# Duankaiwen/LSNet

Hardware: AMD Instinct MI355X
Metric: img/s train LSNet R-50-FPN 1333x800 bs2/GPU (higher is better)
Workload: dtype f32 (fp32-equivalent: 6 bf16 MFMA terms per product on exact 3-way operand splits, fp32 accumulate); 1 GPU; LSNet R50-FPN bbox (conv_module_type=dcn), 2 img/GPU 3x800x1344 (1333x800 padded to /32), 7 gt/img, fwd+bwd+gradient arena (the reducer's buckets, no collective on one rank)+clip35+SGD; global_batch=2, parallelism=dp1, world_size=1, memory_format=channels_last, launch=eager

## Files before the change

### include/lsnet_hip.h

```cpp
#ifndef LSNET_HIP_H_
#define LSNET_HIP_H_

#include <stdint.h>

#ifdef __cplusplus
extern "C" {
#endif

typedef struct ihipStream_t *lsn_stream_t;

typedef enum {
    LSN_OK = 0,
    LSN_ERR_INVALID = -1,
    LSN_ERR_UNSUPPORTED = -2,
    LSN_ERR_RUNTIME = -3
} lsn_status;

typedef enum { LSN_NCHW = 0, LSN_NHWC = 1 } lsn_layout;

typedef struct { int64_t b, c, h, w; } lsn_strides4;

typedef struct {
    int B, C, H, W;
    int Co, Ho, Wo;
    int kh, kw, stride, pad, dil;
    int groups, deformable_groups;
    float scale_h, scale_w;
    int mask_is_logit;
    void *workspace;
    void *gather_workspace;
    int64_t gather_workspace_bytes;
    int accumulate_param_grads;
    int out_pitch;
    int weights_prepared;
} lsn_dcn_shape;

typedef struct {
    const float *input;
    const float *offset;
    const float *mask;
    float *output;
    const float *grad_output;
    float *grad_input;
    float *grad_offset;
    float *grad_mask;
    lsn_strides4 off_st, mask_st;
    int B, H, W, Ho, Wo;
    float scale_h, scale_w;
} lsn_dcn_level;

const char *lsn_last_error(void);
int lsn_version(void);

enum { LSN_MATH_FP32 = 0, LSN_MATH_BF16X3 = 1, LSN_MATH_BF16X6 = 2, LSN_MATH_BF16 = 3 };
int lsn_set_math_mode(int mode);
int lsn_get_math_mode(void);


#define LSN_DCN_KD_EVERY_ROUTE 55

int lsn_dcn_forward(const lsn_dcn_shape *shape, int n_levels, const lsn_dcn_level *levels,
                    const float *weight, const float *bias, lsn_layout layout, lsn_stream_t stream);

int lsn_dcn_backward(const lsn_dcn_shape *shape, int n_levels, const lsn_dcn_level *levels,
                     const float *weight, float *grad_weight, float *grad_bias, lsn_layout layout,
                     lsn_stream_t stream);

int64_t lsn_dcn_backward_workspace_bytes(const lsn_dcn_shape *shape, int n_levels, const lsn_dcn_level *levels);
int lsn_dcn_pitched_ok(const lsn_dcn_shape *shape, int n_levels, const lsn_dcn_level *levels, int backward);
int lsn_dcn_prepared_ok(const lsn_dcn_shape *shape, int n_levels, const lsn_dcn_level *levels, int backward);
int lsn_dcn_anchor_lists(const lsn_dcn_shape *shape, int n_levels, const lsn_dcn_level *levels, lsn_layout layout,
                         int *sample_anchor, int *list_start, int *list_sample, int64_t *counts, lsn_stream_t stream);


int lsn_deform_conv_forward(const float *input, const float *weight, const float *offset, float *output,
                            int B, int C, int H, int W, int Co, int kW, int kH, int dW, int dH, int padW,
                            int padH, int dilW, int dilH, int group, int deformable_group,
                            int im2col_step, lsn_stream_t stream);
int lsn_deform_conv_backward_input(const float *input, const float *offset, const float *grad_output,
                                   float *grad_input, float *grad_offset, const float *weight, int B,
                                   int C, int H, int W, int Co, int kW, int kH, int dW, int dH, int padW,
                                   int padH, int dilW, int dilH, int group, int deformable_group,
                                   int im2col_step, lsn_stream_t stream);
int lsn_deform_conv_backward_parameters(const float *input, const float *offset, const float *grad_output,
                                        float *grad_weight, int B, int C, int H, int W, int Co, int kW,
                                        int kH, int dW, int dH, int padW, int padH, int dilW, int dilH,
                                        int group, int deformable_group, float scale, int im2col_step,
                                        lsn_stream_t stream);
int lsn_modulated_deform_conv_forward(const float *input, const float *weight, const float *bias,
                                      const float *offset, const float *mask, float *output, int B, int C,
                                      int H, int W, int Co, int kernel_h, int kernel_w, int stride_h,
                                      int stride_w, int pad_h, int pad_w, int dilation_h, int dilation_w,
                                      int group, int deformable_group, int with_bias, lsn_stream_t stream);
int lsn_modulated_deform_conv_backward(const float *input, const float *weight, const float *bias,
                                       const float *offset, const float *mask, float *grad_input,
                                       float *grad_weight, float *grad_bias, float *grad_offset,
                                       float *grad_mask, const float *grad_output, int B, int C, int H,
                                       int W, int Co, int kernel_h, int kernel_w, int stride_h,
                                       int stride_w, int pad_h, int pad_w, int dilation_h, int dilation_w,
                                       int group, int deformable_group, int with_bias,
                                       lsn_stream_t stream);
int lsn_pyramid_deform_conv_forward(const float *input, const float *weight, const float *offset,
                                    float *output, int B, int C, int H, int W, int Co, int Ho, int Wo,
                                    int kW, int kH, int dW, int dH, int padW, int padH, int dilW, int dilH,
                                    float scaleW, float scaleH, int group, int deformable_group,
                                    int im2col_step, lsn_stream_t stream);
int lsn_pyramid_deform_conv_backward_input(const float *input, const float *offset,
                                           const float *grad_output, float *grad_input,
                                           float *grad_offset, const float *weight, int B, int C, int H,
                                           int W, int Co, int Ho, int Wo, int kW, int kH, int dW, int dH,
                                           int padW, int padH, int dilW, int dilH, float scaleW,
                                           float scaleH, int group, int deformable_group,
                                           int im2col_step, lsn_stream_t stream);
int lsn_pyramid_deform_conv_backward_parameters(const float *input, const float *offset,
                                                const float *grad_output, float *grad_weight, int B,
                                                int C, int H, int W, int Co, int Ho, int Wo, int kW,
                                                int kH, int dW, int dH, int padW, int padH, int dilW,
                                                int dilH, float scaleW, float scaleH, int group,
                                                int deformable_group, float scale, int im2col_step,
                                                lsn_stream_t stream);

int lsn_sigmoid_focal_loss_forward(const float *logits, const int64_t *targets, float *losses, int N,
                                   int C, float gamma, float alpha, lsn_stream_t stream);
// ... 344 lines not shown
```

### lsnet_amd/_lib.py

```python
import ctypes
import os

_HERE = os.path.dirname(os.path.abspath(__file__))
SO_PATH = os.environ.get('LSNET_HIP_SO') or os.path.join(_HERE, 'csrc', 'liblsnet_hip.so')


class Strides4(ctypes.Structure):
    c_name = 'lsn_strides4'
    _fields_ = [('b', ctypes.c_int64), ('c', ctypes.c_int64), ('h', ctypes.c_int64), ('w', ctypes.c_int64)]


class DcnShape(ctypes.Structure):
    c_name = 'lsn_dcn_shape'
    _fields_ = [('B', ctypes.c_int), ('C', ctypes.c_int), ('H', ctypes.c_int), ('W', ctypes.c_int),
                ('Co', ctypes.c_int), ('Ho', ctypes.c_int), ('Wo', ctypes.c_int),
                ('kh', ctypes.c_int), ('kw', ctypes.c_int), ('stride', ctypes.c_int), ('pad', ctypes.c_int),
                ('dil', ctypes.c_int), ('groups', ctypes.c_int), ('deformable_groups', ctypes.c_int),
                ('scale_h', ctypes.c_float), ('scale_w', ctypes.c_float), ('mask_is_logit', ctypes.c_int),
                ('workspace', ctypes.c_void_p), ('gather_workspace', ctypes.c_void_p),
                ('gather_workspace_bytes', ctypes.c_int64), ('accumulate_param_grads', ctypes.c_int),
                ('out_pitch', ctypes.c_int), ('weights_prepared', ctypes.c_int)]


class DcnLevel(ctypes.Structure):
    c_name = 'lsn_dcn_level'
    _fields_ = [('input', ctypes.c_void_p), ('offset', ctypes.c_void_p), ('mask', ctypes.c_void_p),
                ('output', ctypes.c_void_p), ('grad_output', ctypes.c_void_p), ('grad_input', ctypes.c_void_p),
                ('grad_offset', ctypes.c_void_p), ('grad_mask', ctypes.c_void_p),
                ('off_st', Strides4), ('mask_st', Strides4),
                ('B', ctypes.c_int), ('H', ctypes.c_int), ('W', ctypes.c_int), ('Ho', ctypes.c_int),
                ('Wo', ctypes.c_int), ('scale_h', ctypes.c_float), ('scale_w', ctypes.c_float)]


class OffsetChainLevel(ctypes.Structure):
    c_name = 'lsn_offset_chain_level'
    _fields_ = [('off', ctypes.c_void_p), ('out', ctypes.c_void_p * 3), ('gout', ctypes.c_void_p * 6), ('goff', ctypes.c_void_p),
                ('images', ctypes.c_int64), ('per_image', ctypes.c_int64), ('off_image_pitch', ctypes.c_int64),
                ('mh', ctypes.c_float * 3), ('mw', ctypes.c_float * 3)]


class WgradBnJob(ctypes.Structure):
    c_name = 'lsn_wgrad_bn_job'
    _fields_ = [('x', ctypes.c_void_p), ('g', ctypes.c_void_p), ('w', ctypes.c_void_p), ('bn_gamma', ctypes.c_void_p),
                ('bn_mean', ctypes.c_void_p), ('bn_var', ctypes.c_void_p), ('bn_eps', ctypes.c_float),
                ('grad_w', ctypes.c_void_p), ('grad_gamma', ctypes.c_void_p), ('grad_beta', ctypes.c_void_p)]


class SgdTensor(ctypes.Structure):
    c_name = 'lsn_sgd_tensor'
    _fields_ = [('param', ctypes.c_void_p), ('grad', ctypes.c_void_p), ('momentum_buf', ctypes.c_void_p),
                ('numel', ctypes.c_int64), ('first_chunk', ctypes.c_int64), ('group', ctypes.c_int)]


class SgdGroup(ctypes.Structure):
    c_name = 'lsn_sgd_group'
    _fields_ = [('lr', ctypes.c_float), ('momentum', ctypes.c_float), ('weight_decay', ctypes.c_float)]


class ConvLevel(ctypes.Structure):
    c_name = 'lsn_conv_level'
    _fields_ = [('x', ctypes.c_void_p), ('out', ctypes.c_void_p), ('grad_out', ctypes.c_void_p),
                ('B', ctypes.c_int), ('H', ctypes.c_int), ('W', ctypes.c_int), ('residual', ctypes.c_void_p),
                ('gate', ctypes.c_void_p)]


class ConvWprep(ctypes.Structure):
    c_name = 'lsn_conv_wprep'
    _fields_ = [('kind', ctypes.c_int), ('w', ctypes.c_void_p), ('prepared', ctypes.c_void_p), ('C', ctypes.c_int),
                ('Co', ctypes.c_int), ('kh', ctypes.c_int), ('kw', ctypes.c_int), ('stride', ctypes.c_int),
                ('pad', ctypes.c_int), ('dil', ctypes.c_int),
                ('bn_gamma', ctypes.c_void_p), ('bn_var', ctypes.c_void_p), ('bn_beta', ctypes.c_void_p),
                ('bn_mean', ctypes.c_void_p), ('shift_out', ctypes.c_void_p), ('bn_eps', ctypes.c_float)]


class GnLevel(ctypes.Structure):
    c_name = 'lsn_gn_level'
    _fields_ = [('x', ctypes.c_void_p), ('y', ctypes.c_void_p), ('dy', ctypes.c_void_p), ('dx', ctypes.c_void_p),
                ('B', ctypes.c_int), ('HW', ctypes.c_int), ('y_batch_stride', ctypes.c_longlong),
                ('dy_batch_stride', ctypes.c_longlong)]


class GateJob(ctypes.Structure):
    c_name = 'lsn_gate_job'
    _fields_ = [('grad_y', ctypes.c_void_p), ('y', ctypes.c_void_p), ('grad', ctypes.c_void_p), ('B', ctypes.c_int),
# ... 8 lines not shown


class DecodeSource(ctypes.Structure):
    c_name = 'lsn_decode_source'
    _fields_ = [('H', ctypes.c_int), ('W', ctypes.c_int), ('stride', ctypes.c_float),
                ('heat', ctypes.c_void_p), ('offset', ctypes.c_void_p),
                ('heat_strides', ctypes.c_int64 * 4), ('offset_strides', ctypes.c_int64 * 4)]


class CornerLevel(ctypes.Structure):
    c_name = 'lsn_corner_level'
    _fields_ = [('H', ctypes.c_int), ('W', ctypes.c_int), ('score', ctypes.c_void_p), ('offset', ctypes.c_void_p),
                ('score_strides', ctypes.c_int64 * 4), ('offset_strides', ctypes.c_int64 * 4),
                ('grad_score', ctypes.c_void_p), ('grad_offset', ctypes.c_void_p),
                ('grad_score_strides', ctypes.c_int64 * 4), ('grad_offset_strides', ctypes.c_int64 * 4)]


class SemLevel(ctypes.Structure):
    c_name = 'lsn_sem_level'
    _fields_ = [('H', ctypes.c_int), ('W', ctypes.c_int), ('logits', ctypes.c_void_p), ('strides', ctypes.c_int64 * 4),
                ('grad', ctypes.c_void_p), ('grad_strides', ctypes.c_int64 * 4)]


class ProfEntry(ctypes.Structure):
    c_name = 'lsn_prof_entry'
    _fields_ = [('name', ctypes.c_char * 48), ('launches', ctypes.c_longlong), ('total_ms', ctypes.c_double),
                ('flops', ctypes.c_double), ('bytes', ctypes.c_double)]


class ProfLaunch(ctypes.Structure):
    c_name = 'lsn_prof_launch'
    _fields_ = [(k, ctypes.c_int) for k in ('kind', 'C', 'Co', 'kh', 'kw', 'stride', 'pad', 'dil', 'relu', 'xpitch', 'n_levels',
                                            'has_residual', 'has_gate')] + \
               [('B', ctypes.c_int * 16), ('H', ctypes.c_int * 16), ('W', ctypes.c_int * 16), ('ms', ctypes.c_float)]


STRUCTS = (Strides4, DcnShape, DcnLevel, OffsetChainLevel, WgradBnJob, SgdTensor, SgdGroup, ConvLevel, ConvWprep, GnLevel, GateJob,
           DecodeLevel, DecodeSource, CornerLevel, SemLevel, ProfEntry, ProfLaunch)


def _signatures():
    i, q, f, d, p, c_char_p, P = ctypes.c_int, ctypes.c_int64, ctypes.c_float, ctypes.c_double, ctypes.c_void_p, \
        ctypes.c_char_p, ctypes.POINTER
    return {
        'lsn_last_error': (c_char_p, []),
        'lsn_version': (i, []),
        'lsn_set_math_mode': (i, [i]),
        'lsn_get_math_mode': (i, []),
        'lsn_dcn_forward': (i, [P(DcnShape), i, P(DcnLevel), p, p, i, p]),
        'lsn_dcn_backward': (i, [P(DcnShape), i, P(DcnLevel), p, p, p, i, p]),
        'lsn_dcn_backward_workspace_bytes': (q, [P(DcnShape), i, P(DcnLevel)]),
        'lsn_dcn_pitched_ok': (i, [P(DcnShape), i, P(DcnLevel), i]),
        'lsn_dcn_prepared_ok': (i, [P(DcnShape), i, P(DcnLevel), i]),
        'lsn_dcn_anchor_lists': (i, [P(DcnShape), i, P(DcnLevel), i, p, p, p, p, p]),
        'lsn_deform_conv_forward': (i, [p] * 4 + [i] * 16 + [p]),
        'lsn_deform_conv_backward_input': (i, [p] * 6 + [i] * 16 + [p]),
        'lsn_deform_conv_backward_parameters': (i, [p] * 4 + [i] * 15 + [f, i, p]),
        'lsn_modulated_deform_conv_forward': (i, [p] * 6 + [i] * 16 + [p]),
        'lsn_modulated_deform_conv_backward': (i, [p] * 11 + [i] * 16 + [p]),
        'lsn_pyramid_deform_conv_forward': (i, [p] * 4 + [i] * 15 + [f, f, i, i, i, p]),
        'lsn_pyramid_deform_conv_backward_input': (i, [p] * 6 + [i] * 15 + [f, f, i, i, i, p]),
        'lsn_pyramid_deform_conv_backward_parameters': (i, [p] * 4 + [i] * 15 + [f, f, i, i, f, i, p]),
        'lsn_sigmoid_focal_loss_forward': (i, [p, p, p, i, i, f, f, p]),
        'lsn_sigmoid_focal_loss_backward': (i, [p] * 4 + [i, i, f, f, p]),
        'lsn_sigmoid_focal_loss_sum': (i, [p] * 4 + [i, i, f, f, p]),
        'lsn_sigmoid_focal_loss_backward_weighted': (i, [p] * 5 + [i, i, f, f, p]),
        'lsn_sigmoid_focal_loss_level_sums': (i, [p] * 4 + [i] * 4 + [p, f, f, p]),
        'lsn_sigmoid_focal_loss_backward_levels': (i, [p] * 5 + [i] * 4 + [p, f, f, p]),
        'lsn_level_sums': (i, [p, p, i, i, i, p, p]),
        'lsn_level_expand': (i, [p, p, i, i, i, p, p]),
        'lsn_clip_sgd_workspace_bytes': (q, []),
        'lsn_clip_sgd_step': (i, [i, p, q, i, P(SgdGroup), f, p, p, p]),
        'lsn_offset_chain_forward': (i, [i, P(OffsetChainLevel), i, p]),
        'lsn_offset_chain_backward': (i, [i, P(OffsetChainLevel), i, p]),
        'lsn_topk_columns': (i, [p] + [i] * 4 + [p, p, i, i, p, p, p]),
        'lsn_assign_workspace_bytes': (q, [i] * 4),
        'lsn_centroid_assign': (i, [p, i, p, p, i, f, i] + [p] * 5),
        'lsn_centroid_assign_batch': (i, [p, i, p, p, i, p, f, i] + [p] * 5),
        'lsn_atss_assign': (i, [p, i, i, i, p, p, i, i] + [p] * 6),
        'lsn_atss_assign_batch': (i, [p, i, i, i, p, p, i, p, i] + [p] * 6),
        'lsn_dense_targets': (i, [p, i, p, i, p, p]),
        'lsn_centroid_assign_masked_batch': (i, [p, i, p, p, p, i, p, f, i] + [p] * 5),
        'lsn_atss_assign_masked_batch': (i, [p, i, i, i, p, p, p, i, p, i] + [p] * 6),
        'lsn_assign_targets_batch': (i, [p, p, i, i, p, p, i, p, q] + [p] * 6),
        'lsn_nms_workspace_bytes': (q, [i]),
        'lsn_nms': (i, [p, p, i, f] + [p] * 4),
        'lsn_conv2d_prepared_bytes': (q, [i] * 8),
        'lsn_conv2d_prepare_weights': (i, [i, p, p] + [i] * 7 + [p]),
        'lsn_conv2d_prepare_weights_multi': (i, [i, P(ConvWprep), p]),
        'lsn_conv2d_prepare_weights_item': (i, [P(ConvWprep), p]),
        'lsn_conv2d_forward_prepared': (i, [i, P(ConvLevel), p, p] + [i] * 9 + [p]),
        'lsn_conv2d_backward_data_prepared': (i, [i, P(ConvLevel), p] + [i] * 7 + [p]),
        'lsn_conv2d_forward': (i, [p] * 5 + [i] * 11 + [p]),
        'lsn_conv2d_forward_multi': (i, [i, P(ConvLevel), p, p, p] + [i] * 8 + [p]),
        'lsn_conv2d_backward_data_multi': (i, [i, P(ConvLevel), p, p] + [i] * 7 + [p]),
        'lsn_conv2d_backward_weight_multi': (i, [i, P(ConvLevel), p, p] + [i] * 8 + [p]),
        'lsn_conv2d_forward_pitched': (i, [p] * 5 + [i] * 12 + [p]),
        'lsn_conv2d_backward_data': (i, [p] * 4 + [i] * 10 + [p]),
        'lsn_conv2d_backward_weight': (i, [p] * 4 + [i] * 11 + [p]),
        'lsn_conv2d_backward_weight_bn': (i, [p] * 6 + [f, p, p, p] + [i] * 11 + [p]),
        'lsn_conv2d_backward_weight_bn_jobs': (i, [i, P(WgradBnJob)] + [i] * 11 + [p]),
        'lsn_grouped_conv2d_forward': (i, [p] * 4 + [i] * 12 + [p]),
        'lsn_grouped_conv2d_backward_data': (i, [p, p, p] + [i] * 11 + [p]),
        'lsn_grouped_conv2d_backward_weight': (i, [p] * 4 + [i] * 12 + [p]),
        'lsn_group_norm_workspace_bytes': (q, [i, P(GnLevel), i, i]),
        'lsn_group_norm_forward': (i, [i, P(GnLevel), i, i, p, p, f, i, p, p, p]),
# ... 159 lines not shown
```

### lsnet_amd/csrc/dcn.hip

```cpp
#include <limits.h>
#include <string.h>

#include <vector>

#include "conv_route.h"
#include "dcn_kernels.h"
#include "dcn_mm_kernels.h"
#include "dcn_grouped_kernels.h"
#include "dcn_route.h"
#include "lib_state.h"
#include "prof.h"

namespace lsn {

static long long *g_dbg_buf = nullptr;
static int g_dbg_block = 0;
static bool dbg_on(int bit) { return (g_dbg_block & bit) != 0; }

static double dcn_flops(const DcnArgs &a)
{
    double px = 0;
    for (int i = 0; i < a.nlv; ++i) px += (double)a.lv[i].B * a.lv[i].Ho * a.lv[i].Wo;
    return 2.0 * px * a.Co * (a.C / a.groups) * a.kh * a.kw;
}
// ... 236 lines not shown
    dim3 grid(a.ntiles, cdiv(Cog, BN), a.groups);
    return vec ? launch256(dcn_fwd_kernel<BM, BN, WM, WN, true>, grid, lds, st, a)
               : launch256(dcn_fwd_kernel<BM, BN, WM, WN, false>, grid, lds, st, a);
}

static int launch_forward_grouped(const DcnArgs &a_in, hipStream_t st)
{
    DcnArgs a = a_in;
    a.ntiles = number_tiles(a, GF_PX);
    ProfScope prof(PROF_FWD, a, st);
    const size_t lds = dcn_fwd_grouped_lds_bytes(a.kh * a.kw);
    const dim3 grid(a.ntiles * (a.C / GF_CH));
    switch (a.C / a.groups) {
    case 8: return launch256(dcn_fwd_grouped_kernel<8>, grid, lds, st, a);
    case 16: return launch256(dcn_fwd_grouped_kernel<16>, grid, lds, st, a);
    default: return launch256(dcn_fwd_grouped_kernel<32>, grid, lds, st, a);
    }
}

static int launch_forward_fp32(const DcnArgs &a, int bn, bool vec, hipStream_t st)
{
    ProfScope prof(PROF_FWD, a, st);
    return bn == 64 ? launch_forward_t<64, 64, 2, 2>(a, vec, st) : launch_forward_t<64, 256, 1, 4>(a, vec, st);
}

static int launch_forward_xn(const DcnArgs &a, bool planes, hipStream_t st)
{
    dim3 grid(a.ntiles, cdiv(a.Co / a.groups, PIPE_BN), a.groups);
    ProfScope prof(PROF_FWD, a, st);
    return split_dispatch(math_np(), [&](auto npc) {
        constexpr int NP = decltype(npc)::value;
        const size_t ldsn = xn_lds_bytes<NP>(a.kh * a.kw * a.dg);
        return planes ? launch256(dcn_fwd_xn_kernel<true, NP>, grid, ldsn, st, a) : launch256(dcn_fwd_xn_kernel<false, NP>, grid, ldsn, st, a);
    });
}

template <int RED>
static int launch_bwd_data_t(const DcnArgs &a, bool vec, hipStream_t st)
{
    const int KD = a.kh * a.kw * a.dg;
    const size_t lds = bwd_fp32_lds(RED, KD);
    return vec ? launch256(dcn_bwd_data_kernel<RED, true>, dim3(a.ntiles), lds, st, a)
               : launch256(dcn_bwd_data_kernel<RED, false>, dim3(a.ntiles), lds, st, a);
}

static_assert(DR_MAXLV == MAXLV && DR_GT == GT && DR_GF_CH == GF_CH && DR_GC_COLS == GC_COLS, "dcn_route.h plans for these kernels");
static_assert(DR_WG_BP == WG_BP && DR_WG_BN == WG_BN && DR_WG_BM == WG_BM, "dcn_route.h counts the steps and tiles of these kernels");
static_assert(DR_TAP_BYTES == sizeof(Tap) && DR_GENTRY_BYTES == sizeof(GEntry), "dcn_route.h sizes the tables of these kernels");
static_assert(DR_FP32_BM == BWD_BM, "dcn_route.h sizes the tap tables of the fp32 kernels");

static size_t gather_ws_bytes(const lsn_dcn_shape &s) { return (size_t)(s.gather_workspace_bytes > 0 ? s.gather_workspace_bytes : 0); }
static bool aligned16(const void *p) { return (reinterpret_cast<uintptr_t>(p) & 15) == 0; }

static DcnRouteShape route_shape(const DcnArgs &a, const lsn_dcn_shape &s, lsn_layout layout, bool want_wgrad)
{
    DcnRouteShape r = {};
    r.n = a.nlv;
    for (int i = 0; i < a.nlv; ++i) {
        const Lvl &L = a.lv[i];
        DcnRouteLevel &R = r.lv[i];
        R.B = L.B, R.H = L.H, R.W = L.W, R.Ho = L.Ho, R.Wo = L.Wo, R.P = L.P;
        R.gx = L.gx != nullptr, R.goff = L.goff != nullptr, R.gmsk = L.gmsk != nullptr;
        R.x_aligned16 = aligned16(L.x), R.gout_aligned16 = aligned16(L.gout);
        R.gx_id = 0;
        while (a.lv[R.gx_id].gx != L.gx) ++R.gx_id;
    }
    const int K = a.kh * a.kw, KD = K * a.dg;
    r.C = a.C, r.Co = a.Co, r.kh = a.kh, r.kw = a.kw, r.groups = a.groups, r.dg = a.dg, r.SL = a.SL, r.opitch = a.opitch;
    r.np = math_np(), r.npl = split_npl(r.np);
    r.nchw = layout == LSN_NCHW, r.want_wgrad = want_wgrad;
    r.workspace = s.workspace != nullptr;
    r.gather_ws = s.gather_workspace != nullptr, r.gather_ws_bytes = gather_ws_bytes(s);
    r.gather_ws_aligned16 = aligned16(s.gather_workspace);
    r.general_gemms = dbg_on(LSN_DBG_GENERAL_GEMMS), r.atomic_scatter = dbg_on(LSN_DBG_ATOMIC_SCATTER);
    r.anchor_one_wave = dbg_on(LSN_DBG_ANCHOR_ONE_WAVE);
    r.fwd_mm_lds = dcn_fwd_mm_lds_bytes(r.npl, KD), r.xn_lds = xn_lds_bytes(r.npl, KD), r.bwd_xn_lds = bwd_xn_lds_bytes(r.np, KD);
    r.fwd_grouped_lds = dcn_fwd_grouped_lds_bytes(K);
    r.wfrag_fwd = cv_wfrag_bytes(a.Co, K, a.C, r.npl), r.wfrag_bwd = cv_wfrag_bytes(K * a.C, 1, a.Co, r.npl);
    return r;
}

static void bind_plan(DcnArgs &a, const GatherPlan &pl, GatherArgs &ga, AnchorArgs &aa)
{
    for (int i = 0; i < a.nlv; ++i) a.lv[i].prow0 = pl.prow0[i], a.lv[i].abase = pl.abase[i];
    const int K = a.kh * a.kw, KD = K * a.dg;
    ga.ng = pl.nblk, ga.NB = pl.NB, ga.C = a.C, ga.K = K, ga.KD = KD, ga.dg = a.dg;
    aa.ng = pl.nanc, aa.NA = pl.NA, aa.C = a.C, aa.K = K, aa.KD = KD, aa.dg = a.dg;
    aa.ncb = pl.ncb, aa.hb_slot = pl.hb_slot;
    for (int j = 0; j < pl.nblk; ++j) {
        const GatherPlanGroup &G = pl.blk[j];
        ga.g[j] = GatherGrp{a.lv[G.level].gx, a.lv[G.level].x, G.B, G.H, G.W, G.abase, G.first};
    }
    for (int j = 0; j < pl.nanc; ++j) {
        const GatherPlanGroup &G = pl.anc[j];
        aa.g[j] = AnchorGrp{a.lv[G.level].gx, a.lv[G.level].x, G.B, G.H, G.W, G.abase, G.first};
    }
}

static void bind_nhwc(DcnArgs &a, int n, const lsn_dcn_level *lv)
{
    for (int i = 0; i < n; ++i) a.lv[i].x = lv[i].input, a.lv[i].gout = lv[i].grad_output, a.lv[i].gx = lv[i].grad_input;
}

static int bwd_tap_groups(const DcnArgs &a)
{
    const int K = a.kh * a.kw;
    int best = 1;
    double best_cost = 1e30;
    for (int g = 1; g <= K; ++g) {
        if (K % g) continue;
        const double cost = (double)cdiv(a.ntiles * g, 512) / g * (1.0 + 0.05 * g);
        if (cost < best_cost - 1e-9) best_cost = cost, best = g;
    }
    return best;
}

struct SideStream {
    hipStream_t side = nullptr;
    hipEvent_t fork = nullptr, join = nullptr;
};
static PerStream<SideStream> g_side;
static int side_stream(hipStream_t st, SideStream **out)
{
    return g_side.get(st, "side streams", out, [&](SideStream &S) {
        if (int rc = refuse_capture(st, "side stream would be created")) return rc;
        int lo = 0, hi = 0;
        LSN_HIP(hipDeviceGetStreamPriorityRange(&lo, &hi));
        LSN_HIP(hipStreamCreateWithPriority(&S.side, hipStreamNonBlocking, hi));
        LSN_HIP(hipEventCreateWithFlags(&S.fork, hipEventDisableTiming));
        LSN_HIP(hipEventCreateWithFlags(&S.join, hipEventDisableTiming));
        return 0;
    });
}

static int build_lists(DcnArgs &a, const GatherPlan &pl, unsigned char *ws, hipStream_t st)
{
    int *hist = reinterpret_cast<int *>(ws + pl.o_hist), *start = reinterpret_cast<int *>(ws + pl.o_start);
    int *key = reinterpret_cast<int *>(ws + pl.o_key);
    int2 *pairs[2] = {reinterpret_cast<int2 *>(ws + pl.o_pairs), reinterpret_cast<int2 *>(ws + pl.o_pairs) + pl.nsamples};
    GEntry *ent = reinterpret_cast<GEntry *>(ws + pl.o_ent);
    Tap *gtap = reinterpret_cast<Tap *>(ws + pl.o_gtap);
    const int KD = a.kh * a.kw * a.dg, n = pl.nsamples, na = pl.nanchors;
    a.gtap_rows = n / KD;
    const int db = ds_digit_bits(na), passes = ds_passes(na), nblocks = ds_blocks(n);
    const dim3 grid(nblocks), block(DS_THREADS), kblock(DS_KEY_THREADS);
    const size_t lds = ds_scatter_lds_bytes(db);
    hipLaunchKernelGGL(dcn_list_keys_kernel, grid, kblock, 0, st, a, n, na, db, nblocks, key, hist, gtap);
    a.gtap = gtap;
// ... 363 lines not shown
    case FWD_XN_PLANES: rc = launch_forward_xn(a, true, st); break;
    case FWD_XN: rc = launch_forward_xn(a, false, st); break;
    case FWD_FP32: rc = launch_forward_fp32(a, r.fp32_bn, r.vec, st); break;
    }
    if (rc) return rc;
    if (layout == LSN_NCHW)
        for (int i = 0; i < n; ++i)
            if (int rc = permute_rs(out_tmp[i], lv[i].output, lv[i].B, lv[i].Ho * lv[i].Wo, s.Co, st)) return rc;
    return 0;
}

static int dcn_backward_impl(const lsn_dcn_shape &s, int n, const lsn_dcn_level *lv, const float *weight,
                             float *grad_weight, float *grad_bias, lsn_layout layout, hipStream_t st)
{
    if (int rc = check_shape(s)) return rc;
    LSN_CHECK(weight != nullptr, "weight is NULL");
    if (grad_bias && !grad_weight)
        return fail(LSN_ERR_UNSUPPORTED, "grad_bias without grad_weight is not supported");
    DcnArgs a;
    if (int rc = fill_levels(a, s, n, lv, BWD_BM)) return rc;
    Scratch ws(st);
    const int K = s.kh * s.kw, Cg = s.C / s.groups;
    std::vector<float *> gx_tmp(n, nullptr), x_tmp(n, nullptr), go_tmp(n, nullptr);
    float *gw_tmp = nullptr, *w_tmp = nullptr;
    for (int i = 0; i < n; ++i) LSN_CHECK(lv[i].input && lv[i].grad_output, "level %d: input/grad_output is NULL", i);
    if (layout == LSN_NHWC) {
        a.w = weight;
        a.gw = grad_weight;
        bind_nhwc(a, n, lv);
    } else {
        w_tmp = ws.get((size_t)s.Co * Cg * K);
        if (!w_tmp) return fail(LSN_ERR_RUNTIME, "workspace allocation failed");
        a.w = w_tmp;
        if (grad_weight) {
            gw_tmp = ws.get((size_t)s.Co * Cg * K);
            if (!gw_tmp) return fail(LSN_ERR_RUNTIME, "workspace allocation failed");
            a.gw = gw_tmp;
        }
        for (int i = 0; i < n; ++i) {
            x_tmp[i] = ws.get(n_in(s, lv[i])), go_tmp[i] = ws.get(n_out(s, lv[i]));
            if (!x_tmp[i] || !go_tmp[i]) return fail(LSN_ERR_RUNTIME, "workspace allocation failed");
            a.lv[i].x = x_tmp[i];
            a.lv[i].gout = go_tmp[i];
            if (lv[i].grad_input) {
                gx_tmp[i] = ws.get(n_in(s, lv[i]));
                if (!gx_tmp[i]) return fail(LSN_ERR_RUNTIME, "workspace allocation failed");
                a.lv[i].gx = gx_tmp[i];
            }
        }
    }
    a.gb = grad_bias;

    void *gws = s.gather_workspace;
    const DcnRoute r = route_backward(route_shape(a, s, layout, a.gw != nullptr));
    if (r.lds_over)
        return fail(LSN_ERR_UNSUPPORTED, "deformable backward: kh*kw*deformable_groups = %d needs %zu B of LDS (> 160 KiB) in the "
                    "fp32 scatter kernel, the only one left for this call; every call with at most %d is served",
                    K * s.deformable_groups, r.lds_over, DCN_KD_EVERY_ROUTE);
    if (a.opitch != a.Co && r.data == DATA_NONE)
        return fail(LSN_ERR_UNSUPPORTED, "deformable backward: out_pitch without a data-gradient pass");
    if (a.opitch != a.Co && !r.pitched)
        return fail(LSN_ERR_UNSUPPORTED, "deformable backward: out_pitch %d != Co %d outside the matrix-pipe kernels "
                    "(lsn_dcn_pitched_ok)", a.opitch, a.Co);
    if (s.weights_prepared && r.data != DATA_NONE && !r.prepared)
        return fail(LSN_ERR_UNSUPPORTED, "deformable backward: weights_prepared outside the matrix-pipe kernels (lsn_dcn_prepared_ok)");
    if (layout == LSN_NCHW) {
        if (int rc = permute_rs(weight, w_tmp, s.Co, Cg, K, st)) return rc;
        for (int i = 0; i < n; ++i) {
            if (int rc = permute_rs(lv[i].input, x_tmp[i], lv[i].B, s.C, lv[i].H * lv[i].W, st)) return rc;
            if (int rc = permute_rs(lv[i].grad_output, go_tmp[i], lv[i].B, s.Co, lv[i].Ho * lv[i].Wo, st)) return rc;
        }
    }
    if (r.data != DATA_NONE) {
        if (r.own_gather_ws && !(gws = ws.get(r.plan.bytes / 4 + 64)))
            return fail(LSN_ERR_RUNTIME, "workspace allocation failed");
        if (int rc = prepare_image(a, r.image, s, true, st)) return rc;
        if (int rc = launch_bwd_data(a, r, gws, st)) return rc;
    }
    if (r.wgrad != WG_NONE)
        if (int rc = launch_wgrad(a, r, s.accumulate_param_grads != 0 && layout == LSN_NHWC, st)) return rc;
    if (layout == LSN_NCHW) {
        for (int i = 0; i < n; ++i)
            if (gx_tmp[i])
                if (int rc = permute_rs(gx_tmp[i], lv[i].grad_input, lv[i].B, lv[i].H * lv[i].W, s.C, st)) return rc;
        if (gw_tmp)
            if (int rc = permute_rs(gw_tmp, grad_weight, s.Co, K, Cg, st)) return rc;
    }
    return 0;
}

static lsn_strides4 nchw_strides(int Ch, int H, int W)
{
    lsn_strides4 s;
    s.b = (int64_t)Ch * H * W;
    s.c = (int64_t)H * W;
    s.h = W;
    s.w = 1;
    return s;
}

static int make_single(lsn_dcn_shape &s, lsn_dcn_level &L, int B, int C, int H, int W, int Co, int Ho, int Wo,
                       int kH, int kW, int dH, int dW, int padH, int padW, int dilH, int dilW, int group, int dg,
                       float scaleH, float scaleW, bool pyramid)
{
    if (dH != dW || padH != padW || dilH != dilW)
        return fail(LSN_ERR_UNSUPPORTED, "different stride/pad/dilation for h and w is not supported");
    memset(&s, 0, sizeof(s));
// ... 86 lines not shown
{
    LSN_CHECK(c.s.fold_jobs <= 1, "conv2d backward-weight: folded-norm jobs share a launch on the patch kernel only");
    DcnArgs a;
    const int steps = conv_dcn_args(a, c);
    a.wg_vec = wgrad_vec_bits(a);
    return split_dispatch(c.s.np == 0 ? 6 : c.s.np, [&](auto npc) {
        constexpr int NP = decltype(npc)::value;
        return a.Co <= 64 ? conv_wgrad_launch<NP, 64>(a, steps, c, st) : conv_wgrad_launch<NP, 256>(a, steps, c, st);
    });
}

}

using namespace lsn;

extern "C" {

int lsn_debug_phase_clocks(long long *device_buf_512, int word)
{
    constexpr int known = LSN_DBG_BLOCK_MASK | LSN_DBG_ANCHOR_ONE_WAVE | LSN_DBG_FWD_SK_ALWAYS | LSN_DBG_FWD_SK_NEVER |
                          LSN_DBG_ATOMIC_SCATTER | LSN_DBG_WG_COMPUTED_TAPS | LSN_DBG_WG_SCALAR_LOADS | LSN_DBG_GENERAL_GEMMS;
    if (word & ~known) return fail(LSN_ERR_INVALID, "lsn_debug_phase_clocks: unknown debug bits 0x%x", (unsigned)(word & ~known));
    lsn::g_dbg_buf = device_buf_512;
    lsn::g_dbg_block = word;
    return 0;
}

static bool query_shape(DcnRouteShape &rs, const lsn_dcn_shape *shape, int n_levels, const lsn_dcn_level *levels, int backward,
                        bool want_wgrad)
{
    using namespace lsn;
    DcnArgs a;
    if (!shape || !levels || check_shape(*shape) != 0) return false;
    if (fill_levels(a, *shape, n_levels, levels, backward ? BWD_BM : 64) != 0) return false;
    bind_nhwc(a, n_levels, levels);
    rs = route_shape(a, *shape, LSN_NHWC, want_wgrad);
    return true;
}

int64_t lsn_dcn_backward_workspace_bytes(const lsn_dcn_shape *shape, int n_levels, const lsn_dcn_level *levels)
{
    DcnRouteShape rs;
    if (!query_shape(rs, shape, n_levels, levels, 1, false)) return 0;
    rs.workspace = rs.gather_ws = true, rs.gather_ws_bytes = SIZE_MAX;
    const DcnRoute r = route_backward(rs);
    return r.gather() ? (int64_t)r.plan.bytes : 0;
}

int lsn_dcn_prepared_ok(const lsn_dcn_shape *shape, int n_levels, const lsn_dcn_level *levels, int backward)
{
    DcnRouteShape rs;
    if (!query_shape(rs, shape, n_levels, levels, backward, false)) return 0;
    return (backward ? route_backward(rs) : route_forward(rs)).prepared ? 1 : 0;
}

int lsn_dcn_pitched_ok(const lsn_dcn_shape *shape, int n_levels, const lsn_dcn_level *levels, int backward)
{
    DcnRouteShape rs;
    if (!query_shape(rs, shape, n_levels, levels, backward, true)) return 0;
    return (backward ? route_backward(rs) : route_forward(rs)).pitched ? 1 : 0;
}

int lsn_dcn_anchor_lists(const lsn_dcn_shape *shape, int n_levels, const lsn_dcn_level *levels, lsn_layout layout,
                         int *sample_anchor, int *list_start, int *list_sample, int64_t *counts, lsn_stream_t stream)
{
    using namespace lsn;
    if (!shape || !levels || !counts) return fail(LSN_ERR_INVALID, "shape/levels/counts is NULL");
    const lsn_dcn_shape &s = *shape;
    hipStream_t st = reinterpret_cast<hipStream_t>(stream);
    if (int rc = check_shape(s)) return rc;
    DcnArgs a;
    if (layout != LSN_NHWC) return fail(LSN_ERR_UNSUPPORTED, "lsn_dcn_anchor_lists: LSN_NHWC only");
    if (int rc = fill_levels(a, s, n_levels, levels, BWD_BM)) return rc;
    for (int i = 0; i < n_levels; ++i) LSN_CHECK(levels[i].input && levels[i].grad_output, "level %d: input/grad_output is NULL", i);
    bind_nhwc(a, n_levels, levels);
    const DcnRoute r = route_backward(route_shape(a, s, layout, false));
    if (!r.gather()) return fail(LSN_ERR_UNSUPPORTED, "lsn_dcn_anchor_lists: this call builds no anchor lists (route without the gather pass)");
    const GatherPlan &pl = r.plan;
    counts[0] = pl.nsamples, counts[1] = pl.nanchors;
    if (!sample_anchor && !list_start && !list_sample) return 0;
    LSN_CHECK(sample_anchor && list_start && list_sample, "lsn_dcn_anchor_lists: all three outputs or none");
    unsigned char *w = reinterpret_cast<unsigned char *>(s.gather_workspace);
    GatherArgs ga;
    AnchorArgs aa;
    bind_plan(a, pl, ga, aa);
    if (int rc = build_lists(a, pl, w, st)) return rc;
    const int n = pl.nsamples > pl.nanchors + 1 ? pl.nsamples : pl.nanchors + 1;
    hipLaunchKernelGGL(dcn_list_export_kernel, dim3(cdiv(n, 256)), dim3(256), 0, st, pl.nsamples, pl.nanchors,
                       reinterpret_cast<const int *>(w + pl.o_key), reinterpret_cast<const int *>(w + pl.o_start),
                       reinterpret_cast<const GEntry *>(w + pl.o_ent), sample_anchor, list_start, list_sample);
    LSN_HIP(hipGetLastError());
    return 0;
}

int lsn_dcn_forward(const lsn_dcn_shape *shape, int n_levels, const lsn_dcn_level *levels, const float *weight,
                    const float *bias, lsn_layout layout, lsn_stream_t stream)
{
    if (!shape || !levels) return fail(LSN_ERR_INVALID, "shape/levels is NULL");
    return dcn_forward_impl(*shape, n_levels, levels, weight, bias, layout, stream);
}

int lsn_dcn_backward(const lsn_dcn_shape *shape, int n_levels, const lsn_dcn_level *levels, const float *weight,
                     float *grad_weight, float *grad_bias, lsn_layout layout, lsn_stream_t stream)
{
    if (!shape || !levels) return fail(LSN_ERR_INVALID, "shape/levels is NULL");
    return dcn_backward_impl(*shape, n_levels, levels, weight, grad_weight, grad_bias, layout, stream);
// ... 147 lines not shown
```

### lsnet_amd/csrc/dcn_gather_kernels.h

```cpp
#pragma once
#include "dcn_sort_plan.h"

namespace lsn {

struct __align__(16) GEntry {
    int s;
    int pad;
    float ly, lx;
};

struct GatherGrp {
    float *gx;
    const float *x;
    int B, H, W;
    int abase;
    int blk0;
};
struct GatherArgs {
    GatherGrp g[MAXLV];
    int ng, NB;
    int C, K, KD, dg;
    const float *gcol;
    const int *start;
    const GEntry *ent;
    int raw;
    float *Hb;
};

struct AnchorGrp {
    float *gx;
    const float *x;
    int B, H, W;
    int abase;
    int a0;
};
struct AnchorArgs {
    AnchorGrp g[MAXLV];
    int ng, NA;
    int C, K, KD, dg;
    const float *gcol;
    const int *start;
    const GEntry *ent;
    float *S;
    int raw;
    float *Hb;
    int ncb;
    long long hb_slot;
};

template <int CTRL>
__device__ __forceinline__ float dpp_f32(float v)
{
    return __int_as_float(__builtin_amdgcn_update_dpp(0, __float_as_int(v), CTRL, 0xf, 0xf, true));
}
__device__ __forceinline__ float wave64_sum16(const float (&d)[16], int lane)
{
    const bool b0 = lane & 1, b1 = lane & 2, b2 = lane & 4, b3 = lane & 8;
    float w[8], w2[4], z[2];
#pragma unroll
    for (int i = 0; i < 8; ++i) w[i] = (b0 ? d[2 * i + 1] : d[2 * i]) + dpp_f32<0xB1>(b0 ? d[2 * i] : d[2 * i + 1]);
#pragma unroll
    for (int i = 0; i < 4; ++i) w2[i] = (b1 ? w[2 * i + 1] : w[2 * i]) + dpp_f32<0x4E>(b1 ? w[2 * i] : w[2 * i + 1]);
#pragma unroll
    for (int i = 0; i < 2; ++i) z[i] = (b2 ? w2[2 * i + 1] : w2[2 * i]) + dpp_f32<0x124>(b2 ? w2[2 * i] : w2[2 * i + 1]);
    float r = (b3 ? z[1] : z[0]) + dpp_f32<0x128>(b3 ? z[0] : z[1]);
    r += __shfl_xor(r, 16);
    r += __shfl_xor(r, 32);
    return r;
}

__device__ __forceinline__ const Lvl &find_level_by_row(const DcnArgs &a, int prow)
{
    int li = 0;
    while (li + 1 < a.nlv && prow >= a.lv[li + 1].prow0) ++li;
    return a.lv[li];
}

__global__ __launch_bounds__(256) void dcn_gcol_grouped_kernel(const DcnArgs a, long long nquads)
{
    const int K = a.kh * a.kw, C = a.C, Cg = C / a.groups, Cog = a.Co / a.groups, C4 = C >> 2;
    for (long long id = blockIdx.x * (long long)blockDim.x + threadIdx.x; id < nquads; id += (long long)gridDim.x * blockDim.x) {
        const long long row = id / C4;
        const int c = (int)(id - row * C4) * 4;
        const int prow = (int)(row / K), k = (int)(row - (long long)prow * K);
        const Lvl &L = find_level_by_row(a, prow);
        const int g = c / Cg, ci = c - g * Cg;
        const float *go = L.gout + (size_t)(prow - L.prow0) * a.Co + (size_t)g * Cog;
// ... 321 lines not shown
                        for (int dy = 0; dy < 2; ++dy)
#pragma unroll
                            for (int dx = 0; dx < 2; ++dx) {
                                const float w = ((dy ? ly[u] : hy) * (dx ? lx[u] : hx)) * mm[u];
                                S[dy][dx].x += w * v[u].x, S[dy][dx].y += w * v[u].y;
                                S[dy][dx].z += w * v[u].z, S[dy][dx].w += w * v[u].w;
                            }
                    }
                    if (ga.Hb != nullptr) {
                        float d[16];
                        unsigned okm = 0;
#pragma unroll
                        for (int u = 0; u < GU; ++u)
#pragma unroll
                            for (int q = 0; q < 4; ++q) {
                                d[u * 4 + q] = v[u].x * xa[q >> 1][q & 1].x + v[u].y * xa[q >> 1][q & 1].y +
                                               v[u].z * xa[q >> 1][q & 1].z + v[u].w * xa[q >> 1][q & 1].w;
                                if (j0 + u < n && inb[q >> 1][q & 1]) okm |= 1u << (u * 4 + q);
                            }
                        const float tot = wave64_sum16(d, lane);
                        const int su = __shfl(e.s, min(j0 + ((lane >> 2) & 3), n - 1));
                        if (lane < 16 && ((okm >> lane) & 1u)) {
                            float *hp = ga.Hb + (size_t)su * 4 + (lane & 3);
                            *hp = cb == 0 ? tot : *hp + tot;
                        }
                    }
                }
            }
#pragma unroll
            for (int dy = 0; dy < 2; ++dy)
#pragma unroll
                for (int dx = 0; dx < 2; ++dx)
                    if (inb[dy][dx]) {
                        float4 *ap = &acc[(ai - 1 + dy) * GT + (aj - 1 + dx)][lane];
                        float4 t = *ap;
                        t.x += S[dy][dx].x, t.y += S[dy][dx].y, t.z += S[dy][dx].z, t.w += S[dy][dx].w;
                        *ap = t;
                    }
        }
        if constexpr (NW == 4) __syncthreads();
        if (wave == 0 && c < C) {
#pragma unroll
            for (int i = 0; i < GT; ++i)
#pragma unroll
                for (int j = 0; j < GT; ++j)
                    if (y0 + i < G.H && x0 + j < G.W) {
                        float4 r = acc[i * GT + j][lane];
                        if constexpr (NW == 4) {
                            const float4 r1 = accs[1][i * GT + j][lane], r2 = accs[2][i * GT + j][lane],
                                         r3 = accs[3][i * GT + j][lane];
                            r.x = (r.x + r2.x) + (r1.x + r3.x), r.y = (r.y + r2.y) + (r1.y + r3.y);
                            r.z = (r.z + r2.z) + (r1.z + r3.z), r.w = (r.w + r2.w) + (r1.w + r3.w);
                        }
                        *reinterpret_cast<float4 *>(G.gx + ((size_t)(b * G.H + y0 + i) * G.W + x0 + j) * C + c) = r;
                    }
        }
        if constexpr (NW == 4) __syncthreads();
    }
}

template <int NW>
__global__ __launch_bounds__(256) void dcn_anchor_sum_kernel(const AnchorArgs ga, int a_begin, int a_count)
{
    constexpr int GU = 4;
    __shared__ float4 red[NW == 4 ? 2 : 1][NW == 4 ? 4 : 1][NW == 4 ? 64 : 1];
    const int lane = threadIdx.x & 63, wave_id = threadIdx.x >> 6;
    const int wave = NW == 4 ? wave_id : 0;
    const int C = ga.C, K = ga.K, KD = ga.KD, cpdg = C / ga.dg;
    const int aidx = NW == 4 ? xcd_remap(blockIdx.x, gridDim.x) : xcd_remap(blockIdx.x, gridDim.x) * 4 + wave_id;
    if (aidx >= a_count) return;
    const int ai = a_begin + aidx;
    int gi = 0;
    while (gi + 1 < ga.ng && ai >= ga.g[gi + 1].a0) ++gi;
    const AnchorGrp &G = ga.g[gi];
    const int an = G.abase + (ai - G.a0);
    const int lb = ga.start[an], le = ga.start[an + 1];
    const int la = ai - G.a0, ab = la / ((G.H + 1) * (G.W + 1)), arem = la - ab * (G.H + 1) * (G.W + 1);
    const int ay = arem / (G.W + 1) - 1, ax = arem % (G.W + 1) - 1;
    const int cb0 = ga.ncb > 1 ? (int)blockIdx.y * 256 : 0, cb1 = ga.ncb > 1 ? min(cb0 + 256, C) : C;
    float *const Hbase = ga.Hb != nullptr ? ga.Hb + (size_t)(ga.ncb > 1 ? blockIdx.y : 0) * ga.hb_slot : nullptr;
    for (int cb = cb0; cb < cb1; cb += 256) {
        const int c = cb + lane * 4;
        float4 acc[2][2];
#pragma unroll
        for (int i = 0; i < 2; ++i)
#pragma unroll
            for (int j = 0; j < 2; ++j) acc[i][j] = make_float4(0.f, 0.f, 0.f, 0.f);
        float4 xq[2][2];
        bool qin[2][2];
#pragma unroll
        for (int i = 0; i < 2; ++i)
#pragma unroll
            for (int j = 0; j < 2; ++j) {
                qin[i][j] = ay + i >= 0 && ay + i < G.H && ax + j >= 0 && ax + j < G.W;
                xq[i][j] = (ga.Hb != nullptr && qin[i][j] && c < C)
                               ? *reinterpret_cast<const float4 *>(G.x + ((size_t)(ab * G.H + ay + i) * G.W + ax + j) * C + c)
                               : make_float4(0.f, 0.f, 0.f, 0.f);
            }
        for (int base = lb; base < le; base += 64) {
            const int n = min(64, le - base);
            GEntry e = {};
            if (lane < n) e = ga.ent[base + lane];
            for (int j0 = wave * GU; j0 < n; j0 += NW * GU) {
                float4 v[GU];
                float ly[GU], lx[GU], mm[GU];
#pragma unroll
                for (int u = 0; u < GU; ++u) {
// ... 46 lines not shown
            }
        }
        auto put = [&](int slot) __attribute__((always_inline)) {
#pragma unroll
            for (int q = 0; q < 4; ++q) red[slot][q][lane] = acc[q >> 1][q & 1];
        };
        auto add = [&](int slot) __attribute__((always_inline)) {
#pragma unroll
            for (int q = 0; q < 4; ++q) {
                const float4 r = red[slot][q][lane];
                acc[q >> 1][q & 1].x += r.x, acc[q >> 1][q & 1].y += r.y, acc[q >> 1][q & 1].z += r.z, acc[q >> 1][q & 1].w += r.w;
            }
        };
        if constexpr (NW == 4) {
            if (wave >= 2) put(wave - 2);
            __syncthreads();
            if (wave < 2) add(wave);
            __syncthreads();
            if (wave == 1) put(0);
            __syncthreads();
            if (wave == 0) add(0);
        }
        if (wave == 0 && c < C) {
#pragma unroll
            for (int q = 0; q < 4; ++q)
                *reinterpret_cast<float4 *>(ga.S + ((size_t)ai * 4 + q) * C + c) = acc[q >> 1][q & 1];
        }
        if constexpr (NW == 4) __syncthreads();
    }
}

__global__ __launch_bounds__(256) void dcn_anchor_combine_kernel(const AnchorArgs ga, int npix)
{
    const int lane = threadIdx.x & 63;
    const int pi = blockIdx.x * 4 + (threadIdx.x >> 6);
    if (pi >= npix) return;
    int gi = 0, p0 = 0;
    while (gi + 1 < ga.ng && pi >= p0 + ga.g[gi].B * ga.g[gi].H * ga.g[gi].W) p0 += ga.g[gi].B * ga.g[gi].H * ga.g[gi].W, ++gi;
    const AnchorGrp &G = ga.g[gi];
    const int lp = pi - p0;
    const int b = lp / (G.H * G.W), rem = lp - b * G.H * G.W;
    const int y = rem / G.W, x = rem - y * G.W;
    auto S = [&](int ay, int ax, int q) -> const float * {
        return ga.S + ((size_t)(G.a0 + (b * (G.H + 1) + ay + 1) * (G.W + 1) + ax + 1) * 4 + q) * ga.C;
    };
    for (int c = lane * 4; c < ga.C; c += 256) {
        const float4 s11 = *reinterpret_cast<const float4 *>(S(y - 1, x - 1, 3) + c);
        const float4 s10 = *reinterpret_cast<const float4 *>(S(y - 1, x, 2) + c);
        const float4 s01 = *reinterpret_cast<const float4 *>(S(y, x - 1, 1) + c);
        const float4 s00 = *reinterpret_cast<const float4 *>(S(y, x, 0) + c);
        float4 r;
        r.x = ((s11.x + s10.x) + s01.x) + s00.x, r.y = ((s11.y + s10.y) + s01.y) + s00.y;
        r.z = ((s11.z + s10.z) + s01.z) + s00.z, r.w = ((s11.w + s10.w) + s01.w) + s00.w;
        *reinterpret_cast<float4 *>(G.gx + ((size_t)(b * G.H + y) * G.W + x) * ga.C + c) = r;
    }
}

__global__ void dcn_offgrad_kernel(const DcnArgs a, int nsamples, const float4 *__restrict__ Hb, int ncb)
{
    const int s = blockIdx.x * blockDim.x + threadIdx.x;
    if (s >= nsamples) return;
    const int K = a.kh * a.kw, KD = K * a.dg;
    const int prow = s / KD, kd = s - prow * KD;
    const int dgi = kd / K, k = kd - dgi * K;
    const Lvl &L = find_level_by_row(a, prow);
    if (L.goff == nullptr && L.gmsk == nullptr) return;
    const Tap tp = a.gtap[(size_t)kd * a.gtap_rows + prow];
    float4 h = make_float4(0.f, 0.f, 0.f, 0.f);
    if (tp.flags) {
        h = Hb[s];
        for (int y = 1; y < ncb; ++y) {
            const float4 t = Hb[(size_t)y * nsamples + s];
            h.x += t.x, h.y += t.y, h.z += t.z, h.w += t.w;
        }
    }
    const float hy = 1.f - tp.ly, hx = 1.f - tp.lx;
    const float v00 = (tp.flags & 1) ? h.x : 0.f, v01 = (tp.flags & 2) ? h.y : 0.f;
    const float v10 = (tp.flags & 4) ? h.z : 0.f, v11 = (tp.flags & 8) ? h.w : 0.f;
    const float dy = hx * (v10 - v00) + tp.lx * (v11 - v01);
    const float dx = hy * (v01 - v00) + tp.ly * (v11 - v10);
    const float bil = hy * hx * v00 + hy * tp.lx * v01 + tp.ly * hx * v10 + tp.ly * tp.lx * v11;
    const int pix = prow - L.prow0;
    const int HWo = L.Ho * L.Wo;
    const int b = pix / HWo, rem = pix - b * HWo;
    const int ho = rem / L.Wo, wo = rem - ho * L.Wo;
    if (L.goff) {
        float *op = L.goff + (size_t)b * L.osb + (size_t)ho * L.osh + (size_t)wo * L.osw;
        op[(size_t)(dgi * 2 * K + 2 * k) * L.osc] = tp.m * dy;
        op[(size_t)(dgi * 2 * K + 2 * k + 1) * L.osc] = tp.m * dx;
    }
    if (L.gmsk) {
        float gmv = bil;
        if (a.msig) gmv *= tp.m * (1.f - tp.m);
        L.gmsk[(size_t)b * L.msb + (size_t)(dgi * K + k) * L.msc + (size_t)ho * L.msh + (size_t)wo * L.msw] = gmv;
    }
}

}
```

### lsnet_amd/csrc/dcn_route.h

```cpp
#pragma once
#include <stddef.h>
#include <stdint.h>

#include "dcn_sort_plan.h"

constexpr int DR_MAXLV = 16;
constexpr int DR_GT = 4;
constexpr int DR_GF_CH = 64, DR_GC_COLS = 64;
constexpr int DR_WG_BP = 32, DR_WG_BN = 64, DR_WG_BM = 256;
constexpr size_t DR_TAP_BYTES = 32, DR_GENTRY_BYTES = 16;
constexpr size_t DR_LDS_MAX = 160 * 1024;
constexpr int DR_FP32_BM = 64;

struct DcnRouteLevel {
    int B, H, W, Ho, Wo;
    int P;
    bool gx, goff, gmsk;
    bool x_aligned16, gout_aligned16;
    int gx_id;
};

struct DcnRouteShape {
    int n;
    DcnRouteLevel lv[DR_MAXLV];
    int C, Co, kh, kw, groups, dg;
    int SL;
    int opitch;
    int np, npl;
    bool nchw;
    bool want_wgrad;
    bool workspace;
    bool gather_ws;
    size_t gather_ws_bytes;
    bool gather_ws_aligned16;
    bool general_gemms;
    bool atomic_scatter;
    bool anchor_one_wave;
    size_t fwd_mm_lds, xn_lds, bwd_xn_lds, fwd_grouped_lds;
    size_t wfrag_fwd, wfrag_bwd;
};

constexpr int dr_cdiv(int a, int b) { return (a + b - 1) / b; }
inline bool fits_i32(int64_t elems, int bytes_per = 1) { return elems * bytes_per < ((int64_t)1 << 31); }
inline int64_t in_elems(const DcnRouteShape &s, int i) { return (int64_t)s.lv[i].B * s.lv[i].H * s.lv[i].W * s.C; }
inline int64_t col_elems(const DcnRouteShape &s, int i) { return (int64_t)s.lv[i].P * s.kh * s.kw * s.C; }

inline bool vec_ok(const DcnRouteShape &s)
{
    const int Cg = s.C / s.groups, Cog = s.Co / s.groups;
    return (Cg % 4 == 0) && (Cog % 4 == 0) && (s.Co % 4 == 0) && (s.SL % 4 == 0);
}

inline bool mm_common_ok(const DcnRouteShape &s)
{
    if (s.np == 0 || s.groups != 1 || s.dg < 1 || s.C % s.dg != 0 || s.general_gemms) return false;
    for (int i = 0; i < s.n; ++i)
        if (!fits_i32(in_elems(s, i), 4) || !fits_i32((int64_t)s.lv[i].P * s.opitch, 4)) return false;
    return true;
}

inline bool mm_fwd_ok(const DcnRouteShape &s)
{
    if (!mm_common_ok(s) || (s.C / s.dg) % 32 != 0 || s.Co % 128 != 0) return false;
    if (s.fwd_mm_lds > 80 * 1024) return false;
    return fits_i32((int64_t)s.wfrag_fwd);
}

inline bool mm_bwd_ok(const DcnRouteShape &s)
{
    if (!mm_common_ok(s) || s.C % 4 != 0 || s.Co % 4 != 0) return false;
    for (int i = 0; i < s.n; ++i)
        if ((s.lv[i].goff || s.lv[i].gmsk) && !s.lv[i].gx) return false;
// ... 16 lines not shown
    return s.Co / s.groups > 64 && fwd_fp32_lds(256, s.kh * s.kw * s.dg) <= DR_LDS_MAX ? 256 : 64;
}
inline int bwd_fp32_red(const DcnRouteShape &s)
{
    return s.Co / s.groups > 64 && bwd_fp32_lds(256, s.kh * s.kw * s.dg) <= DR_LDS_MAX ? 256 : 64;
}

inline bool grouped_inputs_ok(const DcnRouteShape &s)
{
    for (int i = 0; i < s.n; ++i)
        if (!fits_i32(in_elems(s, i)) || !s.lv[i].x_aligned16) return false;
    return true;
}

inline bool grouped_fwd_ok(const DcnRouteShape &s)
{
    if (s.groups <= 1 || s.C % s.groups != 0 || s.Co != s.C) return false;
    const int cg = s.C / s.groups;
    if (!(cg == 8 || cg == 16 || cg == 32) || s.C % DR_GF_CH != 0 || s.C % s.dg != 0 || (s.C / s.dg) % DR_GF_CH != 0) return false;
    return s.fwd_grouped_lds <= 64 * 1024 && grouped_inputs_ok(s);
}

inline bool bwd_offsets_ok(const DcnRouteShape &s)
{
    for (int i = 0; i < s.n; ++i)
        if (!fits_i32(in_elems(s, i), 4) || !fits_i32(col_elems(s, i), 4)) return false;
    return true;
}

inline bool bwd_x3_ok(const DcnRouteShape &s)
{
    if (s.np == 0 || s.groups != 1) return false;
    if (s.Co > 256 || s.Co % 8 != 0 || s.C % 4 != 0) return false;
    if (!fits_i32((int64_t)s.kh * s.kw * s.C * s.Co, 6)) return false;
    if (s.bwd_xn_lds > 80 * 1024) return false;
    return bwd_offsets_ok(s);
}

inline bool bwd_grouped_ok(const DcnRouteShape &s)
{
    if (s.groups <= 1 && s.np != 0) return false;
    if (s.C % s.groups != 0 || s.Co % s.groups != 0 || (s.C / s.groups) % 4 != 0 || s.C % s.dg != 0) return false;
    if ((s.C / s.dg) % 4 != 0 || s.atomic_scatter) return false;
    for (int i = 0; i < s.n; ++i)
        if ((s.lv[i].goff || s.lv[i].gmsk) && !s.lv[i].gx) return false;
    return bwd_offsets_ok(s);
}

struct GatherPlanGroup {
    int level;
    int B, H, W;
    int abase;
    int first;
};

struct GatherPlan {
    bool ok = false;
    int nsamples = 0, nanchors = 0;
    size_t o_gcol = 0, o_hist = 0, o_start = 0, o_key = 0, o_ent = 0, o_gtap = 0, bytes = 0;
    size_t o_S = 0, o_H = 0, o_pairs = 0;
    int prow0[DR_MAXLV] = {}, abase[DR_MAXLV] = {};
    GatherPlanGroup blk[DR_MAXLV] = {};
    int nblk = 0, NB = 0;
    GatherPlanGroup anc[DR_MAXLV] = {};
    int nanc = 0, NA = 0;
    int ncb = 1;
    long long hb_slot = 0;
    int anchor_pixels = 0;
    int na_long = 0;
    int64_t block_samples = 0;
};

inline size_t align256(size_t v) { return (v + 255) & ~(size_t)255; }

inline GatherPlan gather_plan(const DcnRouteShape &s, bool all_anchor)
{
    GatherPlan pl;
    const int K = s.kh * s.kw, KD = K * s.dg;
    int64_t prow = 0, anchors = 0, Q = 0;
    GatherPlanGroup grp[DR_MAXLV];
    int ng = 0;
    int64_t gsamp[DR_MAXLV] = {};
    for (int i = 0; i < s.n; ++i) {
        const DcnRouteLevel &L = s.lv[i];
        pl.prow0[i] = (int)prow;
        prow += L.P;
        if (!L.gx) continue;
        int gi = -1;
        for (int j = 0; j < ng; ++j)
            if (grp[j].level == L.gx_id) gi = j;
        if (gi < 0) {
            gi = ng++;
            grp[gi] = GatherPlanGroup{i, L.B, L.H, L.W, (int)anchors, (int)Q};
            anchors += (int64_t)L.B * (L.H + 1) * (L.W + 1);
            Q += (int64_t)L.B * dr_cdiv(L.H, DR_GT) * dr_cdiv(L.W, DR_GT);
        } else if (grp[gi].B != L.B || grp[gi].H != L.H || grp[gi].W != L.W) {
            return pl;
        }
        pl.abase[i] = grp[gi].abase;
        gsamp[gi] += (int64_t)L.P * KD;
    }
    if (ng == 0) return pl;
    if (prow * KD >= ((int64_t)1 << 30) || anchors >= ((int64_t)1 << 30) || Q >= ((int64_t)1 << 30)) return pl;
    if (s.C % 4 != 0 || (s.C / s.dg) % 4 != 0) return pl;
    pl.nsamples = (int)(prow * KD);
    pl.nanchors = (int)anchors;
    if (ds_digit_bits(pl.nanchors) > DS_MAX_DIGIT_BITS) return pl;
    constexpr int anchor_thr = 400;
    {
        bool to_anchor[DR_MAXLV], is_long[DR_MAXLV];
        int64_t q = 0;
        for (int j = 0; j < ng; ++j) {
            const GatherPlanGroup &G = grp[j];
            const int64_t nblk = (int64_t)G.B * dr_cdiv(G.H, DR_GT) * dr_cdiv(G.W, DR_GT);
            const int64_t nanch = (int64_t)G.B * (G.H + 1) * (G.W + 1);
            to_anchor[j] = all_anchor || (anchor_thr > 0 && gsamp[j] > (int64_t)anchor_thr * nblk);
            constexpr int long_thr = 40;
            is_long[j] = !all_anchor || gsamp[j] > (int64_t)long_thr * nanch;
        }
        for (int pass = 0; pass < 2; ++pass) {
            for (int j = 0; j < ng; ++j) {
                const GatherPlanGroup &G = grp[j];
                if (!to_anchor[j] || is_long[j] != (pass == 0)) continue;
                pl.anc[pl.nanc] = G, pl.anc[pl.nanc++].first = pl.NA;
                pl.NA += G.B * (G.H + 1) * (G.W + 1);
                pl.anchor_pixels += G.B * G.H * G.W;
            }
            if (pass == 0) pl.na_long = pl.NA;
        }
        for (int j = 0; j < ng; ++j) {
            if (to_anchor[j]) continue;
            const GatherPlanGroup &G = grp[j];
            pl.blk[pl.nblk] = G, pl.blk[pl.nblk++].first = (int)q;
            q += (int64_t)G.B * dr_cdiv(G.H, DR_GT) * dr_cdiv(G.W, DR_GT);
            pl.block_samples += gsamp[j];
        }
        Q = q;
    }
    pl.NB = (int)Q;
    size_t o = 0;
    pl.o_gcol = o, o = align256(o + (size_t)prow * K * s.C * sizeof(float));
    pl.o_hist = o, o = align256(o + ds_hist_ints(pl.nsamples, pl.nanchors) * sizeof(int));
    pl.o_start = o, o = align256(o + ((size_t)pl.nanchors + 1) * sizeof(int));
    pl.o_key = o, o = align256(o + (size_t)pl.nsamples * sizeof(int));
    pl.o_ent = o, o = align256(o + (size_t)pl.nsamples * DR_GENTRY_BYTES);
    pl.o_gtap = o, o = align256(o + ((size_t)pl.nsamples + 1) * DR_TAP_BYTES);
    pl.o_S = o, o = align256(o + (size_t)pl.NA * 4 * s.C * sizeof(float));
    const int ncb_max = (pl.NB == 0 && pl.nanc > 0 && s.C > 256) ? dr_cdiv(s.C, 256) : 1;
    pl.ncb = s.anchor_one_wave ? 1 : ncb_max;
    pl.hb_slot = (long long)pl.nsamples * 4;
    pl.o_H = o, o = align256(o + (size_t)pl.nsamples * 4 * sizeof(float) * ncb_max);
    pl.o_pairs = o, o = align256(o + (size_t)pl.nsamples * 2 * 2 * sizeof(int));
    pl.bytes = o;
    pl.ok = true;
    return pl;
}

inline int wgrad_splits(int cols, int per_cu)
{
    const int slots = 256 * per_cu;
    int s = slots / cols;
    return s < 1 ? 1 : s;
}

inline bool mm_wgrad_ok(const DcnRouteShape &s) { return mm_common_ok(s) && s.Co % 256 == 0 && (s.C / s.dg) % 64 == 0; }
inline bool wgrad_mm_image_ok(const DcnRouteShape &s, int nchunks) { return fits_i32((int64_t)nchunks * 2 * (s.Co / 32) * s.npl, 1024); }

inline bool grouped_wgrad_ok(const DcnRouteShape &s)
{
    if (s.groups <= 1 || s.C % s.groups != 0 || s.Co != s.C || s.kh * s.kw > 9) return false;
    const int cg = s.C / s.groups;
    if (!(cg == 4 || cg == 8 || cg == 16 || cg == 32) || ((int64_t)s.C * cg) % 256 != 0 || s.C % s.dg != 0) return false;
    const int nch = cg >= 16 ? cg : 256 / cg;
    if ((s.C / s.dg) % nch != 0 || s.C % nch != 0) return false;
    return grouped_inputs_ok(s);
}

enum FwdKernel { FWD_MM, FWD_GROUPED, FWD_XN_PLANES, FWD_XN, FWD_FP32 };
enum DataKernel { DATA_NONE, GATHER_GROUPED, GATHER_MM, GATHER_XN, SCATTER_XN, SCATTER_FP32 };
enum WgradKernel { WG_NONE, WG_GROUPED, WG_MM, WG_XN_ORDERED, WG_XN_ATOMIC, WG_FP32_ORDERED, WG_FP32_ATOMIC };
enum WeightImage { IMG_NONE, IMG_FRAGMENT, IMG_PLANES, IMG_PLANES_T };

struct DcnRoute {
    FwdKernel fwd = FWD_FP32;
    DataKernel data = DATA_NONE;
    WgradKernel wgrad = WG_NONE;
    WeightImage image = IMG_NONE;
    bool vec = false;
    bool pitched = false;
    bool prepared = false;
    int gcol_ks = 0;
    int wg_steps = 0;
    int wg_ncol = 0, wg_nz = 0, wg_splits = 0;
    bool own_gather_ws = false;
    int fp32_bn = 0;
    int fp32_red = 0;
    size_t lds_over = 0;
    GatherPlan plan;
    bool gather() const { return data == GATHER_GROUPED || data == GATHER_MM || data == GATHER_XN; }
};

inline DcnRoute route_forward(const DcnRouteShape &s)
{
    DcnRoute r;
    r.vec = vec_ok(s);
    if (s.workspace && mm_fwd_ok(s)) {
        r.fwd = FWD_MM, r.image = IMG_FRAGMENT;
    } else if (grouped_fwd_ok(s)) {
        r.fwd = FWD_GROUPED;
    } else if (s.np != 0 && xn_ok(s) && s.xn_lds <= 160 * 1024) {
        r.fwd = FWD_XN;
        if (s.workspace && (s.C / s.groups) % 8 == 0) r.fwd = FWD_XN_PLANES, r.image = IMG_PLANES;
    }
    if (r.fwd == FWD_FP32) {
        r.fp32_bn = fwd_fp32_bn(s);
        const size_t lds = fwd_fp32_lds(r.fp32_bn, s.kh * s.kw * s.dg);
        if (lds > DR_LDS_MAX) r.lds_over = lds;
    }
    r.pitched = r.prepared = !s.nchw && r.fwd == FWD_MM;
    return r;
}

inline int gcol_mfma_ksteps(const DcnRouteShape &s)
{
    const int Cg = s.C / s.groups, Cog = s.Co / s.groups;
    if (s.C % DR_GC_COLS != 0 || s.opitch % 4 != 0) return 0;
    for (int i = 0; i < s.n; ++i)
        if (!s.lv[i].gout_aligned16) return 0;
    if (s.groups == 1) return (s.Co == 64 || s.Co == 128 || s.Co == 256) ? s.Co / 4 : 0;
    return (Cog == Cg && (Cg == 4 || Cg == 8 || Cg == 16 || Cg == 32)) ? (Cg == 32 ? 8 : 4) : 0;
}

inline int wgrad_split_grid(const DcnRouteShape &s, int nsteps, int *ncol, int *nz)
{
    const int K = s.kh * s.kw, Cg = s.C / s.groups, Cog = s.Co / s.groups;
    *ncol = s.groups * K * (Cg / s.SL) * dr_cdiv(s.SL, DR_WG_BN), *nz = dr_cdiv(Cog, DR_WG_BM);
    int n = wgrad_splits(*ncol * *nz, 2);
    if (n > nsteps) n = nsteps;
    if (n < 1) n = 1;
    return n > 65535 ? 65535 : n;
}

inline DcnRoute route_backward(const DcnRouteShape &s)
{
    DcnRoute r;
    r.vec = vec_ok(s);
    const int K = s.kh * s.kw;
    bool any_data = false;
    for (int i = 0; i < s.n; ++i) any_data = any_data || s.lv[i].gx || s.lv[i].goff || s.lv[i].gmsk;
    if (any_data) {
        const bool can_split = s.workspace && s.np && s.groups == 1 && s.Co % 2 == 0;
        const bool grouped = bwd_grouped_ok(s), mm = mm_bwd_ok(s), x3 = can_split && bwd_x3_ok(s);
        const DataKernel cand = s.atomic_scatter                          ? DATA_NONE
                                : grouped                                 ? GATHER_GROUPED
                                : (can_split && mm && bwd_offsets_ok(s)) ? GATHER_MM
                                : x3                                      ? GATHER_XN
                                                                          : DATA_NONE;
        bool fits = false;
        if (cand != DATA_NONE && (s.gather_ws || s.nchw)) {
            r.plan = gather_plan(s, mm || grouped);
            r.own_gather_ws = !s.gather_ws && r.plan.ok;
            fits = r.plan.ok && (r.own_gather_ws || r.plan.bytes <= s.gather_ws_bytes);
        }
        r.data = fits ? cand : x3 ? SCATTER_XN : SCATTER_FP32;
        if (r.data == GATHER_GROUPED) r.gcol_ks = gcol_mfma_ksteps(s);
        if (r.data == SCATTER_FP32) {
            r.fp32_red = bwd_fp32_red(s);
            const size_t lds = bwd_fp32_lds(r.fp32_red, K * s.dg);
            if (lds > DR_LDS_MAX) r.lds_over = lds;
        }
        r.image = r.data == GATHER_MM ? IMG_FRAGMENT : can_split ? IMG_PLANES_T : IMG_NONE;
        r.prepared = !s.nchw && r.data == GATHER_MM;
    }
    if (s.want_wgrad) {
        int64_t rows = 0, steps = 0;
        for (int i = 0; i < s.n; ++i) rows += s.lv[i].P, steps += dr_cdiv(s.lv[i].P, DR_WG_BP);
        r.wg_steps = (int)steps;
        const size_t nW = (size_t)s.Co * K * (s.C / s.groups);
        const bool tap_table = r.gather() && (r.own_gather_ws || s.gather_ws_aligned16);
        if (grouped_wgrad_ok(s) && s.opitch == s.Co && nW % 4 == 0 && rows < ((int64_t)1 << 30)) {
            r.wgrad = WG_GROUPED;
        } else if (mm_wgrad_ok(s) && tap_table && wgrad_mm_image_ok(s, r.wg_steps)) {
            r.wgrad = WG_MM;
        } else {
            r.wg_splits = wgrad_split_grid(s, r.wg_steps, &r.wg_ncol, &r.wg_nz);
            const bool ordered = nW % 4 == 0 && (size_t)r.wg_splits * (nW + s.Co) * sizeof(float) <= ((size_t)256 << 20);
            r.wgrad = s.np ? (ordered ? WG_XN_ORDERED : WG_XN_ATOMIC) : (ordered ? WG_FP32_ORDERED : WG_FP32_ATOMIC);
        }
    }
    r.pitched = !s.nchw && r.data == GATHER_MM && (!s.want_wgrad || r.wgrad == WG_MM);
    return r;
}
```

### lsnet_amd/models/backbones/resnet.py

```python
import math

import torch
import torch.nn as nn
import torch.utils.checkpoint as cp
from torch.nn.modules.batchnorm import _BatchNorm

from ...cnn import build_conv_layer, build_norm_layer, constant_init, kaiming_init
from ...ops.batch_norm import bn_act
from ...ops import resblock
from ...ops.conv import conv_bn_act, conv_bn_act_frozen
from ...ops.pool import avg_pool, max_pool
from ..builder import BACKBONES


def _conv_bn(conv, bn, x, relu, residual=None):
    out = None
    if isinstance(bn, _BatchNorm):
        out = conv_bn_act_frozen(conv, bn, x, relu, residual)
        if out is None:
            out = conv_bn_act(conv, bn, x, relu, residual)
    return out if out is not None else bn_act(bn, conv(x), relu=relu, residual=residual)


def _shortcut(downsample, x):
    if downsample is None:
        return x
    mods = list(downsample)
    if isinstance(mods[-1], _BatchNorm):
        for m in mods[:-2]:
            x = avg_pool(x, m) if isinstance(m, nn.AvgPool2d) else m(x)
        if len(mods) >= 2:
            return _conv_bn(mods[-2], mods[-1], x, relu=False)
        return bn_act(mods[-1], x, relu=False)
    return downsample(x)


class BasicBlock(nn.Module):
    expansion = 1

    def __init__(self, inplanes, planes, stride=1, dilation=1, downsample=None, style='pytorch', with_cp=False,
                 conv_cfg=None, norm_cfg=dict(type='BN'), dcn=None, plugins=None, **_):
        super().__init__()
        assert dcn is None and plugins is None, 'Not implemented yet.'
        self.norm1_name, norm1 = build_norm_layer(norm_cfg, planes, postfix=1)
        self.norm2_name, norm2 = build_norm_layer(norm_cfg, planes, postfix=2)
        self.conv1 = build_conv_layer(conv_cfg, inplanes, planes, 3, stride=stride, padding=dilation,
                                      dilation=dilation, bias=False)
        self.add_module(self.norm1_name, norm1)
        self.conv2 = build_conv_layer(conv_cfg, planes, planes, 3, padding=1, bias=False)
        self.add_module(self.norm2_name, norm2)
        self.relu = nn.ReLU(inplace=True)
        self.downsample, self.stride, self.dilation, self.with_cp = downsample, stride, dilation, with_cp

    norm1 = property(lambda self: getattr(self, self.norm1_name))
    norm2 = property(lambda self: getattr(self, self.norm2_name))

    def _body(self, x):
        out = _conv_bn(self.conv1, self.norm1, x, relu=True)
        return _conv_bn(self.conv2, self.norm2, out, relu=True, residual=_shortcut(self.downsample, x))

    def forward(self, x):
        return cp.checkpoint(self._body, x) if (self.with_cp and x.requires_grad) else self._body(x)

# ... 169 lines not shown

    def make_res_layer(self, **kwargs):
        return ResLayer(**kwargs)

    norm1 = property(lambda self: getattr(self, self.norm1_name))

    def _freeze_stages(self):
        frozen = []
        if self.frozen_stages >= 0:
            if self.deep_stem:
                self.stem.eval()
                frozen.append(self.stem)
            else:
                self.norm1.eval()
                frozen += [self.conv1, self.norm1]
        for i in range(1, self.frozen_stages + 1):
            m = getattr(self, f'layer{i}')
            m.eval()
            frozen.append(m)
        for m in frozen:
            for p in m.parameters():
                p.requires_grad = False

    def init_weights(self, pretrained=None):
        if isinstance(pretrained, str):
            from ...runner.checkpoint import load_checkpoint
            load_checkpoint(self, pretrained, strict=False)
            return
        if pretrained is not None:
            raise TypeError('pretrained must be a str or None')
        for m in self.modules():
            if isinstance(m, nn.Conv2d):
                kaiming_init(m)
            elif isinstance(m, (_BatchNorm, nn.GroupNorm)):
                constant_init(m, 1)
        if self.dcn is not None:
            for m in self.modules():
                if isinstance(m, Bottleneck) and hasattr(getattr(m, 'conv2', None), 'conv_offset'):
                    constant_init(m.conv2.conv_offset, 0)
        if self.zero_init_residual:
            for m in self.modules():
                if isinstance(m, Bottleneck):
                    constant_init(m.norm3, 0)
                elif isinstance(m, BasicBlock):
                    constant_init(m.norm2, 0)

    def forward(self, x):
        x = self.stem(x) if self.deep_stem else _conv_bn(self.conv1, self.norm1, x, relu=True)
        x = max_pool(x, self.maxpool)
        outs = []
        for i, name in enumerate(self.res_layers):
            x = getattr(self, name)(x)
            if i in self.out_indices:
                outs.append(x)
        return tuple(outs)

    def train(self, mode=True):
        super().train(mode)
        self._freeze_stages()
        if mode and self.norm_eval:
            for m in self.modules():
                if isinstance(m, _BatchNorm):
                    m.eval()
        return self


@BACKBONES.register_module()
class ResNeXt(ResNet):
    arch_settings = {
        50: (Bottleneck, (3, 4, 6, 3)),
        101: (Bottleneck, (3, 4, 23, 3)),
        152: (Bottleneck, (3, 8, 36, 3)),
    }

    def __init__(self, groups=1, base_width=4, **kwargs):
        self.groups, self.base_width = groups, base_width
        super().__init__(**kwargs)

    def make_res_layer(self, **kwargs):
        return ResLayer(groups=self.groups, base_width=self.base_width, base_channels=self.base_channels,
                        **kwargs)
```

### lsnet_amd/models/dense_heads/ls_head.py

```python
import math
import os

import numpy as np
import torch
import torch.nn as nn

from ...cnn import ConvModule, bias_init_with_prob, kaiming_init, normal_init
from ...ops.conv import Conv2d
from ...ops.group_norm import GroupNorm
from ...core import PointGenerator, assigners, build_assigner, build_sampler, multiclass_nms_lsvr
from ...ops.backend import get_backend
from ...ops import ModulatedDeformConvPack, PyramidDeformConv
from ...ops.dcn import offset_scale_chain
from ...ops import cross_iou as fused_ciou
from ...ops import point_decode as point_ops
from ...ops.focal import level_rows_ok, level_sums
from ...ops.streams import side_stream
from ..builder import HEADS, build_loss

FUSED_LEVEL_SUMS = os.environ.get('LSNET_FUSED_LEVEL_SUMS', '1') != '0'
SIDE_STREAM_TARGETS = os.environ.get('LSNET_SIDE_STREAM_TARGETS', '1') != '0'
NATIVE_DECODE = os.environ.get('LSNET_NATIVE_DECODE', '1') != '0'
DECODE_CAND_CAP = 16384

TASK_BRANCHES = {'bbox': ('bbox',), 'segm': ('segm',), 'pose_bbox': ('bbox', 'pose'), 'pose_kbox': ('pose',)}


class DCNConvModule(nn.Module):

    def __init__(self, in_channels=256, out_channels=256, kernel_size=3, dilation=1, num_groups=1, dcn_pad=1):
        super().__init__()
        self.conv = ModulatedDeformConvPack(in_channels, out_channels, kernel_size, 1, dcn_pad)
        self.bn = GroupNorm(num_groups, out_channels)
        self.relu = nn.ReLU(inplace=True)

    def forward(self, x):
        return self.bn.forward_act(self.conv(x))

    def forward_multi(self, xs):
        return self.bn.forward_multi(self.conv.forward_multi(xs), relu=True)


def _split_px_views(x, shapes):
    B, C = x.shape[:2]
    flat = x.permute(0, 2, 3, 1).reshape(B, -1, C)
    outs, o = [], 0
    for h, w in shapes:
        outs.append(flat[:, o:o + h * w].reshape(B, h, w, C).permute(0, 3, 1, 2))
        o += h * w
    return outs


class _SplitPxFn(torch.autograd.Function):

    @staticmethod
    def forward(ctx, x, shapes):
        ctx.shapes, ctx.dims = shapes, (x.shape[0], x.shape[1])
        return tuple(_split_px_views(x, shapes))

    @staticmethod
    def backward(ctx, *grads):
        B, C = ctx.dims
        ref = next(g for g in grads if g is not None)
        parts = [g.permute(0, 2, 3, 1).reshape(B, h * w, C) if g is not None else ref.new_zeros((B, h * w, C))
                 for g, (h, w) in zip(grads, ctx.shapes)]
        flat = torch.cat(parts, dim=1)
# ... 182 lines not shown
        return t[1]

    def _offset_sources(self, branch):
        key = ('offset_sources', branch)
        t = self._consts.get(key)
        if t is None:
            d_init, n_sp = self._out_dims(branch)
            t = self._consts[key] = point_ops.offset_sources(self.task, n_sp, d_init, self.num_kernel_points)
        return t

    @staticmethod
    def _level_list(lvl, num_levels):
        if lvl == 0:
            return [0, 1, 2]
        if lvl == num_levels - 1:
            return [lvl, lvl - 1, lvl - 2]
        return [lvl, lvl - 1, lvl + 1]

    def _gn_cat(self, gn, maps):
        if hasattr(gn, 'forward_cat_px'):
            return gn.forward_cat_px(maps, relu=True)
        return self._cat_px(gn.forward_multi(maps, relu=True))

    @staticmethod
    def _cat_px(maps):
        B, C = maps[0].shape[:2]
        x = torch.cat([m.permute(0, 2, 3, 1).reshape(B, -1, C) for m in maps], dim=1)
        return x.unsqueeze(2).permute(0, 3, 1, 2)

    @staticmethod
    def _split_px(x, shapes):
        if x.requires_grad and torch.is_grad_enabled():
            outs = list(_SplitPxFn.apply(x, tuple(shapes)))
        else:
            outs = _split_px_views(x, shapes)
        for i, o in enumerate(outs):
            o._px_cat = (x, i)
        return outs

    @staticmethod
    def _px_base(maps):
        tags = [getattr(m, '_px_cat', None) for m in maps]
        if any(t is None for t in tags) or any(t[0] is not tags[0][0] or t[1] != i for i, t in enumerate(tags)):
            return None
        x = tags[0][0]
        if sum(m.shape[2] * m.shape[3] for m in maps) != x.shape[2] or x.shape[3] != 1:
            return None
        return x.permute(0, 2, 3, 1).reshape(x.shape[0], x.shape[2], x.shape[1])

    def forward(self, feats, after_init=None):
        nl = len(feats)
        shapes = [tuple(f.shape[2:]) for f in feats]
        base_offset = self._base_offset(feats[0])
        cls_feats = self._run_tower(self.cls_convs, feats)
        st = {}
        for b in self.branches:
            tower = self._run_tower(getattr(self, f'{b}_convs'), feats)
            init_conv, init_out = getattr(self, f'pts_{b}_init_conv'), getattr(self, f'pts_{b}_init_out')
            n_sp = self._out_dims(b)[1]
            raw = init_out(self._cat_px(init_conv.forward_multi(tower, relu=True)))
            if point_ops.native_ok(raw):
                sp, off = point_ops.point_decode(raw, n_sp, self._offset_sources(b), self.gradient_mul, base_offset)
            else:
                sp = self.softplus(raw[:, :n_sp])
                reg = self.get_pred_reg(sp, raw[:, n_sp:] if raw.shape[1] > n_sp else None)
                reg = (1 - self.gradient_mul) * reg.detach() + self.gradient_mul * reg
                off = reg - base_offset
            st[b] = dict(feat=tower, sp_all=sp, sp=self._split_px(sp, shapes), off=self._split_px(off, shapes))

        if after_init is not None:
            after_init({b: st[b]['sp'] for b in self.branches})

        pairs = []
        mults = []
        for l in range(nl):
            bh, bw = cls_feats[l].shape[2:]
            trio = []
            for s in self._level_list(l, nl):
                sh, sw = cls_feats[s].shape[2] / bh, cls_feats[s].shape[3] / bw
                trio.append((sh, sw))
                pairs.append((l, s, sh, sw))
            mults.append(trio)
        driver = self.branches[-1]
        scaled, scaled_cls = {}, None
        for b in self.branches:
            sets = offset_scale_chain(st[b]['off'], mults, copies=2 if b == driver else 1)
            scaled[b] = [t for trio in sets[0] for t in trio]
            if b == driver:
                scaled_cls = [t for trio in sets[1] for t in trio]
        scales = [(p[2], p[3]) for p in pairs]

        def gather(conv, src_feats, offsets):
            return conv.forward_multi([src_feats[p[1]] for p in pairs], offsets, scales, concat=3)

        cls_raw = gather(self.pts_cls_conv, cls_feats, scaled_cls)
        outs = {}
        def fuse(af, fc, raw, feat):
            a = af[0].forward_multi(raw, relu=True)
            if hasattr(fc, 'forward_multi') and 'residuals' in fc.forward_multi.__code__.co_varnames:
                return fc.forward_multi(feat, residuals=a)
            f = fc.forward_multi(feat)
            return [x + y for x, y in zip(a, f)]

        fused = fuse(self.cls_af_dcn_conv, self.cls_feat_conv, cls_raw, cls_feats)
        outs['cls'] = self._split_px(self.pts_cls_out(self._gn_cat(self.cls_GN, fused)), shapes)
        for b in self.branches:
            raw = gather(getattr(self, f'pts_{b}_refine_conv'), st[b]['feat'], scaled[b])
            af, fc = getattr(self, f'{b}_af_dcn_conv'), getattr(self, f'{b}_feat_conv')
            gn, ro = getattr(self, f'{b}_GN'), getattr(self, f'pts_{b}_refine_out')
            fused = fuse(af, fc, raw, st[b]['feat'])
            ref_raw, sp_init = ro(self._gn_cat(gn, fused)), st[b]['sp_all'].detach()
            if point_ops.native_ok(ref_raw, sp_init):
                refine = point_ops.softplus_add(ref_raw, sp_init)
            else:
                refine = self.softplus(ref_raw + sp_init)
            outs[b] = self._split_px(refine, shapes)

        none = [None] * nl
        res = [outs['cls']]
        for b in ('bbox', 'segm', 'pose'):
            res += [st[b]['sp'], outs[b]] if b in self.branches else [none, none]
        return tuple(res)

    def forward_train(self, x, img_metas, gt_bboxes, gt_extremes=None, gt_keypoints=None, gt_masks=None,
                      gt_labels=None, gt_bboxes_ignore=None, proposal_cfg=None, **kwargs):
        pre, stage2, hook = None, [], None
        if SIDE_STREAM_TARGETS and x[0].is_cuda:
            main = torch.cuda.current_stream(x[0].device)
            side = self._side_stream(x[0].device)
            side.wait_stream(main)
            with torch.cuda.stream(side):
                pre = self.init_stage_targets([tuple(f.shape[-2:]) for f in x], x[0], gt_bboxes, gt_extremes, gt_keypoints,
                                              gt_masks, gt_labels, img_metas)

            def hook(init_preds):
                side.wait_stream(main)
                with torch.cuda.stream(side):
                    stage2.append(self.refine_stage_targets(pre, init_preds[self._box_branch()]))
        outs = self(x, after_init=hook)
        if pre is not None:
            main.wait_stream(side)
        losses = self.loss(*outs, gt_bboxes, gt_extremes, gt_keypoints, gt_masks, gt_labels, img_metas,
                           gt_bboxes_ignore=gt_bboxes_ignore, init_stage=pre, refine_stage=stage2[0] if stage2 else None)
        if proposal_cfg is None:
            return losses
        return losses, self.get_bboxes(*outs, img_metas, cfg=proposal_cfg)

    def get_points(self, featmap_sizes, img_metas, device):
        key = ('points', tuple(tuple(s) for s in featmap_sizes), tuple(tuple(m['pad_shape'][:2]) for m in img_metas),
               str(device))
        hit = self._consts.get(key)
        if hit is not None:
            return hit[:3]
        points = [self.point_generators[i].grid_points(featmap_sizes[i], self.point_strides[i], device)
                  for i in range(len(featmap_sizes))]
        flags, counts, all_valid = [], [], True
        for meta in img_metas:
            per_level, per_count = [], []
            h, w = meta['pad_shape'][:2]
            for i, (fh, fw) in enumerate(featmap_sizes):
                s = self.point_strides[i]
                vh, vw = min(int(np.ceil(h / s)), fh), min(int(np.ceil(w / s)), fw)
                all_valid = all_valid and vh == fh and vw == fw
# ... 513 lines not shown
```

### lsnet_amd/models/necks/fpn.py

```python
import torch.nn as nn
import torch.nn.functional as F

from ...cnn import ConvModule, xavier_init
from ...ops.pool import max_pool2d, upsample_add
from ..builder import NECKS


@NECKS.register_module()
class FPN(nn.Module):

    def __init__(self, in_channels, out_channels, num_outs, start_level=0, end_level=-1, add_extra_convs=False,
                 extra_convs_on_inputs=True, relu_before_extra_convs=False, no_norm_on_lateral=False,
                 conv_cfg=None, norm_cfg=None, act_cfg=None, upsample_cfg=dict(mode='nearest')):
        super().__init__()
        assert isinstance(in_channels, (list, tuple))
        self.in_channels, self.out_channels = list(in_channels), out_channels
        self.num_ins, self.num_outs = len(in_channels), num_outs
        self.relu_before_extra_convs = relu_before_extra_convs
        self.no_norm_on_lateral = no_norm_on_lateral
        self.upsample_cfg = dict(upsample_cfg)
        if end_level == -1:
            self.backbone_end_level = self.num_ins
            assert num_outs >= self.num_ins - start_level
        else:
            self.backbone_end_level = end_level
            assert end_level <= self.num_ins
            assert num_outs == end_level - start_level
        self.start_level, self.end_level = start_level, end_level
        assert isinstance(add_extra_convs, (str, bool))
        if isinstance(add_extra_convs, str):
            assert add_extra_convs in ('on_input', 'on_lateral', 'on_output')
        elif add_extra_convs:
            add_extra_convs = 'on_input' if extra_convs_on_inputs else 'on_output'
        self.add_extra_convs = add_extra_convs

        common = dict(conv_cfg=conv_cfg, act_cfg=act_cfg, inplace=False)
        self.lateral_convs = nn.ModuleList(
            ConvModule(self.in_channels[i], out_channels, 1,
                       norm_cfg=None if no_norm_on_lateral else norm_cfg, **common)
            for i in range(start_level, self.backbone_end_level))
        self.fpn_convs = nn.ModuleList(
            ConvModule(out_channels, out_channels, 3, padding=1, norm_cfg=norm_cfg, **common)
            for _ in range(start_level, self.backbone_end_level))
        extra = num_outs - self.backbone_end_level + start_level
        if self.add_extra_convs and extra >= 1:
            for i in range(extra):
                src = self.in_channels[self.backbone_end_level - 1] \
                    if (i == 0 and self.add_extra_convs == 'on_input') else out_channels
                self.fpn_convs.append(ConvModule(src, out_channels, 3, stride=2, padding=1, norm_cfg=norm_cfg,
                                                 **common))

    def init_weights(self):
        for m in self.modules():
            if isinstance(m, nn.Conv2d):
                xavier_init(m, distribution='uniform')

    def forward(self, inputs):
        assert len(inputs) == len(self.in_channels)
        lat = [conv(inputs[i + self.start_level]) for i, conv in enumerate(self.lateral_convs)]
        n = len(lat)
        for i in range(n - 1, 0, -1):
            lat[i - 1] = upsample_add(lat[i], lat[i - 1], self.upsample_cfg)
        outs = [self.fpn_convs[i](lat[i]) for i in range(n)]
        if self.num_outs > n:
            if not self.add_extra_convs:
                for _ in range(self.num_outs - n):
                    outs.append(max_pool2d(outs[-1], 1, stride=2))
            else:
                src = {'on_input': inputs[self.backbone_end_level - 1], 'on_lateral': lat[-1],
                       'on_output': outs[-1]}[self.add_extra_convs]
                outs.append(self.fpn_convs[n](src))
                for i in range(n + 1, self.num_outs):
                    prev = F.relu(outs[-1]) if self.relu_before_extra_convs else outs[-1]
                    outs.append(self.fpn_convs[i](prev))
        return tuple(outs)
```

### lsnet_amd/ops/conv.py

```python
import os

import torch
import torch.nn as nn
import torch.nn.functional as F

from .. import _lib
from .._lib import ptr, stream
from . import grad_sink
from .weight_images import SIDE_STREAM_IMAGES, _fold_bn, invalidate_weight_images, parameters_updated, weight_image

_CL = torch.channels_last


_warned_fallbacks = set()


def _warn_aten_fallback(what, x, detail):
    if not (torch.is_tensor(x) and x.is_cuda):
        return
    key = (what, detail)
    if key in _warned_fallbacks:
        return
    _warned_fallbacks.add(key)
    import warnings
    warnings.warn(f'lsnet_amd.{what}: no HIP kernel of this library serves this call on {x.device} ({detail}); '
                  'falling back to the ATen operator', RuntimeWarning, stacklevel=3)


def _pad_channels(t, c_to, pad=0):
    B, C, H, W = t.shape
    out = t.new_zeros((B, c_to, H + 2 * pad, W + 2 * pad)).contiguous(memory_format=_CL)
    out[:, :C, pad:pad + H, pad:pad + W] = t
    return out


def _pad_in_channels(x, weight, pad=0):
    C4 = (x.shape[1] + 3) // 4 * 4
    return _pad_channels(x, C4, pad), _pad_channels(weight, C4)


def _pad_narrow_co(w, gos):
    Co, C, kh, kw = w.shape
    if not (Co % 4 and C <= 64):
        return w, gos, Co
    Co8 = (Co + 3) // 4 * 4
    gos8 = [_pad_channels(g, Co8) for g in gos]
    w8 = w.new_zeros((Co8, C, kh, kw)).contiguous(memory_format=_CL)
    w8[:Co] = w
    return w8, gos8, Co8


def _out_hw(H, W, kh, kw, stride, pad, dil):
    return (H + 2 * pad - (dil * (kh - 1) + 1)) // stride + 1, (W + 2 * pad - (dil * (kw - 1) + 1)) // stride + 1


def _forward_prepared(x, img, bias, w_shape, stride, pad, dil, relu, residual=None):
    B, C, H, W = x.shape
    Co, _, kh, kw = w_shape
    out = torch.empty((B, Co) + _out_hw(H, W, kh, kw, stride, pad, dil), device=x.device, dtype=torch.float32, memory_format=_CL)
    lv = (_lib.ConvLevel * 1)()
    lv[0].x, lv[0].out, lv[0].B, lv[0].H, lv[0].W, lv[0].residual = ptr(x), ptr(out), B, H, W, ptr(residual)
# ... 48 lines not shown
    B, C, H, W = in_shape
    Co, _, kh, kw = w.shape
    if out is None:
        out = torch.empty(in_shape, device=g.device, dtype=torch.float32, memory_format=_CL)
    lv = (_lib.ConvLevel * 1)()
    lv[0].x, lv[0].out, lv[0].B, lv[0].H, lv[0].W = ptr(g), ptr(out), B, H, W
    lv[0].residual, lv[0].gate = ptr(residual), ptr(gate)
    _lib.check(_lib.load().lsn_conv2d_backward_data_prepared(1, lv, ptr(weight_image(w, 1, stride, pad, dil, bn=bn)), C, Co, kh,
                                                             kw, stride, pad, dil, stream()))
    return out


def wgrad_bn(x, g, w, bn, stride, pad, dil, need=(True, True, True)):
    B, C, H, W = x.shape
    Co, _, kh, kw = w.shape
    gamma, beta = bn.weight, bn.bias
    c = grad_sink.claim(list(zip((w, gamma, beta), need)))
    gw, dg, db = c.sinks if c.accumulate else (torch.empty_like(w), torch.empty_like(gamma), torch.empty_like(beta))
    _lib.check(_lib.load().lsn_conv2d_backward_weight_bn(
        ptr(x), ptr(g), ptr(w), ptr(gamma), ptr(bn.running_mean), ptr(bn.running_var), float(bn.eps), ptr(gw),
        ptr(dg), ptr(db), B, H, W, C, Co, kh, kw, stride, pad, dil, c.accumulate, stream()))
    return c.results((gw, dg, db))


def wgrad_bn_deferrable(w, bn):
    return bool(grad_sink.claim([(w, True), (bn.weight, True), (bn.bias, True)]).accumulate and w.is_cuda)


def wgrad_bn_jobs(jobs, stride, pad, dil):
    x0, _, w0, _ = jobs[0]
    B, C, H, W = x0.shape
    Co, _, kh, kw = w0.shape
    lib = _lib.load()
    claims = [grad_sink.claim([(w, True), (bn.weight, True), (bn.bias, True)]) for _, _, w, bn in jobs]
    assert all(c.accumulate for c in claims), 'wgrad_bn_jobs: a job whose parameters lost their sinks'
    for i in range(0, len(jobs), 8):
        part = jobs[i:i + 8]
        arr = (_lib.WgradBnJob * len(part))()
        for q, (x, g, w, bn), c in zip(arr, part, claims[i:i + 8]):
            assert x.shape == x0.shape and w.shape == w0.shape
            q.x, q.g, q.w = ptr(x), ptr(g), ptr(w)
            q.bn_gamma, q.bn_mean, q.bn_var, q.bn_eps = ptr(bn.weight), ptr(bn.running_mean), ptr(bn.running_var), float(bn.eps)
            q.grad_w, q.grad_gamma, q.grad_beta = map(ptr, c.sinks)
        _lib.check(lib.lsn_conv2d_backward_weight_bn_jobs(len(part), arr, B, H, W, C, Co, kh, kw, stride, pad, dil, 1, stream()))
    for c in claims:
        c.results()


def conv_fwd_bn(x, w, bn, stride, pad, dil, relu, residual=None):
    img, shift = weight_image(w, 0, bn=bn)
    return _forward_prepared(x, img, shift, w.shape, stride, pad, dil, relu, residual)


class _ConvFn(torch.autograd.Function):

    @staticmethod
    def forward(ctx, x, w, bias, stride, pad, dil, relu):
        w = w.contiguous(memory_format=_CL)
        out = _forward_prepared(x, weight_image(w, 0), bias, w.shape, stride, pad, dil, relu)
        ctx.save_for_backward(x, w, out if relu else None)
        ctx.cfg = (stride, pad, dil, relu, bias is not None)
        ctx.bias_ref = bias
        return out

    @staticmethod
    @torch.autograd.function.once_differentiable
    def backward(ctx, go):
        x, w, out = ctx.saved_tensors
        stride, pad, dil, relu, has_bias = ctx.cfg
        lib = _lib.load()
        go = go.contiguous(memory_format=_CL)
        if relu:
            go = relu_gate(go, out) if out.numel() % 4 == 0 else go * (out > 0)
        B, C, H, W = x.shape
        Co, _, kh, kw = w.shape
        gx = gw = gb = None
        if ctx.needs_input_grad[0]:
            w8, (go8,), _ = _pad_narrow_co(w, [go])
            gx = dgrad(go8, w8, x.shape, stride, pad, dil)
        if ctx.needs_input_grad[1] or (has_bias and ctx.needs_input_grad[2]):
            want_b = has_bias and ctx.needs_input_grad[2]
            c, gw, gb = _param_grad_buffers(w, ctx.bias_ref, ctx.needs_input_grad[1], want_b)
            _lib.check(lib.lsn_conv2d_backward_weight(ptr(x), ptr(go), ptr(gw), ptr(gb), B, H, W, C, Co, kh, kw, stride, pad,
                                                      dil, c.accumulate, stream()))
            gw, gb = c.results((gw, gb))
        return gx, gw, gb, None, None, None, None


class _GroupConvFn(torch.autograd.Function):

    @staticmethod
    def forward(ctx, x, w, bias, stride, pad, dil, groups):
        lib = _lib.load()
        B, C, H, W = x.shape
        Co, _, kh, kw = w.shape
        w = w.contiguous(memory_format=_CL)
        out = torch.empty((B, Co) + _out_hw(H, W, kh, kw, stride, pad, dil), device=x.device, dtype=torch.float32, memory_format=_CL)
        _lib.check(lib.lsn_grouped_conv2d_forward(ptr(x), ptr(w), ptr(bias), ptr(out), B, H, W, C, Co, kh, kw, stride, pad, dil,
                                                  groups, 0, stream()))
        ctx.save_for_backward(x, w)
        ctx.cfg = (stride, pad, dil, groups, bias is not None)
        return out

    @staticmethod
    @torch.autograd.function.once_differentiable
    def backward(ctx, go):
        x, w = ctx.saved_tensors
        stride, pad, dil, groups, has_bias = ctx.cfg
        lib = _lib.load()
        go = go.contiguous(memory_format=_CL)
        B, C, H, W = x.shape
        Co, _, kh, kw = w.shape
        gx = gw = gb = None
        if ctx.needs_input_grad[0]:
            gx = torch.empty_like(x, memory_format=_CL)
            _lib.check(lib.lsn_grouped_conv2d_backward_data(ptr(go), ptr(w), ptr(gx), B, H, W, C, Co, kh, kw, stride, pad, dil,
                                                            groups, stream()))
        if ctx.needs_input_grad[1] or (has_bias and ctx.needs_input_grad[2]):
            gw = torch.empty_like(w)
            gb = torch.empty(Co, device=x.device, dtype=torch.float32) if has_bias and ctx.needs_input_grad[2] else None
            _lib.check(lib.lsn_grouped_conv2d_backward_weight(ptr(x), ptr(go), ptr(gw), ptr(gb), B, H, W, C, Co, kh, kw, stride,
                                                              pad, dil, groups, 0, stream()))
            if not ctx.needs_input_grad[1]:
                gw = None
        return gx, gw, gb, None, None, None, None


def hip_group_conv_ok(x, weight, stride, padding, dilation, groups, padding_mode='zeros'):
    if not (x.is_cuda and x.dim() == 4 and x.dtype == torch.float32 and x.is_contiguous(memory_format=_CL)):
        return False
    if groups <= 1 or padding_mode != 'zeros' or isinstance(padding, str):
        return False
    if stride[0] != stride[1] or padding[0] != padding[1] or dilation[0] != dilation[1]:
        return False
    Co, cg, kh, kw = weight.shape
    if x.shape[1] != cg * groups or Co != cg * groups or cg not in (4, 8, 16, 32) or kh * kw > 9:
        return False
    return x.numel() < 2 ** 31 and Co * x.shape[0] * x.shape[2] * x.shape[3] < 2 ** 31


def conv_multi_fwd(xs, w, bias, pad, dil, relu, residuals=None):
    Co, C, kh, kw = w.shape
    n = len(xs)
    levels = (_lib.ConvLevel * n)()
    outs = []
    for i, x in enumerate(xs):
        B, _, H, W = x.shape
        out = torch.empty((B, Co) + _out_hw(H, W, kh, kw, 1, pad, dil), device=x.device, dtype=torch.float32, memory_format=_CL)
        outs.append(out)
        L = levels[i]
        L.x, L.out, L.B, L.H, L.W = ptr(x), ptr(out), B, H, W
        if residuals is not None:
            assert residuals[i].shape == out.shape and residuals[i].is_contiguous(memory_format=_CL)
            L.residual = ptr(residuals[i])
    _lib.check(_lib.load().lsn_conv2d_forward_prepared(n, levels, ptr(weight_image(w, 0)), ptr(bias), C, C, Co, kh, kw, 1, pad, dil,
                                                       1 if relu else 0, stream()))
    return outs


def conv_multi_dgrad(gos, w, xs, pad, dil, accumulate_into=None):
    Co, C, kh, kw = w.shape
    n = len(xs)
    w8, gos8, Co8 = _pad_narrow_co(w, gos)
    levels = (_lib.ConvLevel * n)()
    gxs = []
    for i, x in enumerate(xs):
        gx = accumulate_into[i] if accumulate_into is not None else torch.empty_like(x, memory_format=_CL)
        gxs.append(gx)
        L = levels[i]
        L.x, L.out, L.B, L.H, L.W = ptr(gos8[i]), ptr(gx), x.shape[0], x.shape[2], x.shape[3]
        if accumulate_into is not None:
            L.residual = ptr(gx)
    _lib.check(_lib.load().lsn_conv2d_backward_data_prepared(n, levels, ptr(weight_image(w8, 1, 1, pad, dil)), C, Co8, kh, kw, 1,
                                                             pad, dil, stream()))
    return gxs


def conv_multi_wgrad(xs, gos, w, bias, pad, dil, want_w=True, want_b=True):
    Co, C, kh, kw = w.shape
    n = len(xs)
    levels = (_lib.ConvLevel * n)()
    for i, x in enumerate(xs):
        L = levels[i]
        L.x, L.grad_out, L.B, L.H, L.W = ptr(x), ptr(gos[i]), x.shape[0], x.shape[2], x.shape[3]
    want_b = want_b and bias is not None
    c, gw, gb = _param_grad_buffers(w, bias, want_w, want_b)
    _lib.check(_lib.load().lsn_conv2d_backward_weight_multi(n, levels, ptr(gw), ptr(gb), C, Co, kh, kw, 1, pad, dil, c.accumulate,
                                                            stream()))
    return c.results((gw, gb))


class _ConvMultiFn(torch.autograd.Function):

    @staticmethod
    def forward(ctx, w, bias, cfg, *xs):
        pad, dil, relu = cfg[:3]
        nres = cfg[3] if len(cfg) > 3 else 0
        res = list(xs[len(xs) - nres:]) if nres else None
        xs = xs[:len(xs) - nres] if nres else xs
        w = w.contiguous(memory_format=_CL)
        outs = conv_multi_fwd(xs, w, bias, pad, dil, relu, res)
        ctx.save_for_backward(w, *xs, *(outs if relu else []))
        ctx.cfg, ctx.n, ctx.has_bias, ctx.nres = (pad, dil, relu), len(xs), bias is not None, nres
        ctx.bias_ref = bias
        return tuple(outs)

    @staticmethod
    @torch.autograd.function.once_differentiable
    def backward(ctx, *gos):
        pad, dil, relu = ctx.cfg
        n = ctx.n
        saved = ctx.saved_tensors
        w, xs = saved[0], saved[1:1 + n]
        outs = saved[1 + n:] if relu else None
        if relu and GATE_MULTI:
            gos = relu_gate_multi(list(gos), outs)
        elif relu:
            gos = [g.contiguous(memory_format=_CL) for g in gos]
            gos = [relu_gate(g, o) if o.numel() % 4 == 0 else g * (o > 0) for g, o in zip(gos, outs)]
        else:
            gos = [g.contiguous(memory_format=_CL) for g in gos]
        need_x = [ctx.needs_input_grad[3 + i] for i in range(n)]
        gxs = [None] * n
        if any(need_x):
            gxs = [g if need else None for g, need in zip(conv_multi_dgrad(gos, w, xs, pad, dil), need_x)]
        gw = gb = None
        if ctx.needs_input_grad[0] or (ctx.has_bias and ctx.needs_input_grad[1]):
            gw, gb = conv_multi_wgrad(xs, gos, w, ctx.bias_ref, pad, dil, ctx.needs_input_grad[0],
                                      ctx.has_bias and ctx.needs_input_grad[1])
        gres = [gos[i] if ctx.needs_input_grad[3 + n + i] else None for i in range(ctx.nres)]
        return (gw, gb, None, *gxs, *gres)


def conv2d_multi(xs, weight, bias=None, padding=0, dilation=1, relu=False, residuals=None):
    nres = 0 if residuals is None else len(residuals)
    assert nres in (0, len(xs))
    return list(_ConvMultiFn.apply(weight, bias, (int(padding), int(dilation), bool(relu), nres), *xs, *(residuals or [])))


def hip_conv_ok(x, weight, stride, padding, dilation, groups, padding_mode='zeros'):
    if not (x.is_cuda and x.dim() == 4 and x.dtype == torch.float32):
        return False
    if groups != 1 or padding_mode != 'zeros' or isinstance(padding, str):
        return False
    if stride[0] != stride[1] or padding[0] != padding[1] or dilation[0] != dilation[1]:
        return False
    if x.numel() * 4 >= 2 ** 31 or weight.numel() * 8 >= 2 ** 31 or weight.shape[2] * weight.shape[3] > 64:
        return False
    kh, kw = weight.shape[2], weight.shape[3]
    ho, wo = _out_hw(x.shape[2], x.shape[3], kh, kw, stride[0], padding[0], dilation[0])
    if ho <= 0 or wo <= 0 or x.shape[0] * ho * wo * weight.shape[0] * 4 >= 2 ** 31:
        return False
    return True


def _as_cl(x):
    return x if x.is_contiguous(memory_format=_CL) else x.contiguous(memory_format=_CL)


def _stem_forward(x, weight, bias, stride, pad, relu):
    B, _, H, W = x.shape
    Co, _, kh, kw = weight.shape
    xp, w4 = _pad_in_channels(x, weight, pad)
    C4 = w4.shape[1]
    out = torch.empty((B, Co) + _out_hw(H, W, kh, kw, stride, pad, 1), device=x.device, dtype=torch.float32, memory_format=_CL)
    _lib.check(_lib.load().lsn_conv2d_forward_pitched(ptr(xp), ptr(w4), ptr(bias), ptr(out), None, B, H + 2 * pad, W + 2 * pad,
                                                      kw * C4, C4, Co, kh, 1, stride, 0, 1, 1 if relu else 0, stream()))
    return out


def conv2d(x, weight, bias=None, stride=1, padding=0, dilation=1, relu=False):
    C = x.shape[1]
    no_grad = not (torch.is_grad_enabled() and (x.requires_grad or weight.requires_grad or
                                                (bias is not None and bias.requires_grad)))
    if C < 8 and weight.shape[3] > 1 and int(dilation) == 1 and no_grad:
        return _stem_forward(x, weight, bias, int(stride), int(padding), bool(relu))
    if C % 4:
        x, weight = _pad_in_channels(x, weight)
    return _ConvFn.apply(x, weight, bias, int(stride), int(padding), int(dilation), bool(relu))


def conv_bn_act_frozen(conv, bn, x, relu=True, residual=None):
    if not isinstance(conv, Conv2d) or conv.bias is not None or conv.groups != 1 or bn.training or not bn.affine \
            or not bn.track_running_stats:
        return None
    if conv.weight.requires_grad or bn.weight.requires_grad or bn.bias.requires_grad \
            or (torch.is_grad_enabled() and x.requires_grad):
        return None
    if not hip_conv_ok(x, conv.weight, conv.stride, conv.padding, conv.dilation, conv.groups, conv.padding_mode):
        return None
    x = _as_cl(x)
    w, shift = _fold_bn(conv, bn)
    stride, pad, dil = conv.stride[0], conv.padding[0], conv.dilation[0]
    B, C, H, W = x.shape
    Co, _, kh, kw = w.shape
    if C < 8:
        if residual is not None or kw == 1 or dil != 1:
            return None
        return _stem_forward(x, w, shift, stride, pad, relu)
    if C % 4:
        return None
    if residual is not None:
        if not (tuple(residual.shape) == (B, Co) + _out_hw(H, W, kh, kw, stride, pad, dil) and residual.dtype == torch.float32
                and Co % 4 == 0):
            return None
        residual = _as_cl(residual)
    return _forward_prepared(x, weight_image(w, 0), shift, w.shape, stride, pad, dil, relu, residual)


class _ConvBnActFn(torch.autograd.Function):

    @staticmethod
    def forward(ctx, x, w, gamma, beta, residual, bn, stride, pad, dil, relu):
        out = conv_fwd_bn(x, w, bn, stride, pad, dil, relu, residual)
        ctx.save_for_backward(x, w, out if relu else None)
        ctx.cfg = (stride, pad, dil, relu, residual is not None)
        ctx.bn = bn
        return out

    @staticmethod
    @torch.autograd.function.once_differentiable
    def backward(ctx, gy):
        x, w, y = ctx.saved_tensors
        stride, pad, dil, relu, has_res = ctx.cfg
        bn = ctx.bn
        gy = gy.contiguous(memory_format=_CL)
        need_x, need_w, need_g, need_b = ctx.needs_input_grad[:4]
        need_res = has_res and ctx.needs_input_grad[4]
        g = relu_gate(gy, y) if relu else gy
        gx = gw = dg = db = None
        if need_x:
            gx = dgrad(g, w, x.shape, stride, pad, dil, bn=bn)
        if need_w or need_g or need_b:
            gw, dg, db = wgrad_bn(x, g, w, bn, stride, pad, dil, (need_w, need_g, need_b))
        return gx, gw, dg, db, (g if need_res else None), None, None, None, None, None


def conv_bn_act(conv, bn, x, relu=True, residual=None):
    if not isinstance(conv, Conv2d) or conv.bias is not None or conv.groups != 1 or bn.training or not bn.affine \
            or not bn.track_running_stats or not isinstance(bn, nn.BatchNorm2d):
        return None
    if not hip_conv_ok(x, conv.weight, conv.stride, conv.padding, conv.dilation, conv.groups, conv.padding_mode):
        return None
    Co, C, kh, kw = conv.weight.shape
    if C % 4 or Co % 4 or not (256 % (Co // 4) == 0 if Co <= 1024 else Co % 1024 == 0):
        return None
    if not conv.weight.is_contiguous(memory_format=_CL):
        return None
    x = _as_cl(x)
    stride, pad, dil = conv.stride[0], conv.padding[0], conv.dilation[0]
    B, _, H, W = x.shape
    if residual is not None:
        if not (tuple(residual.shape) == (B, Co) + _out_hw(H, W, kh, kw, stride, pad, dil) and residual.dtype == torch.float32):
            return None
        residual = _as_cl(residual)
    return _ConvBnActFn.apply(x, conv.weight, bn.weight, bn.bias, residual, bn, stride, pad, dil, bool(relu))


class Conv2d(nn.Conv2d):

    def forward(self, x, weight=None):
        if weight is not None:
            return self._run(x, weight)
        return self._run(x, self.weight)

    def forward_multi(self, xs, relu=False, residuals=None):
        xs = list(xs)
        if (1 < len(xs) <= 8 and self.stride[0] == 1 and xs[0].shape[1] % 4 == 0
                and all(hip_conv_ok(x, self.weight, self.stride, self.padding, self.dilation, self.groups,
                                    self.padding_mode) for x in xs)
                and (residuals is None or (self.weight.shape[0] % 4 == 0 and all(r.is_cuda and r.dtype == torch.float32 for r in residuals)))):
            res = None if residuals is None else [_as_cl(r) for r in residuals]
            return conv2d_multi([_as_cl(x) for x in xs], self.weight, self.bias, self.padding[0], self.dilation[0], relu, res)
        outs = [self._run(x, self.weight) for x in xs]
        if residuals is not None:
            outs = [o + r for o, r in zip(outs, residuals)]
        return [F.relu(o) for o in outs] if relu else outs

    def _run(self, x, w):
        if hip_conv_ok(x, w, self.stride, self.padding, self.dilation, self.groups, self.padding_mode):
            return conv2d(_as_cl(x), w, self.bias, self.stride[0], self.padding[0], self.dilation[0], False)
        if hip_group_conv_ok(x, w, self.stride, self.padding, self.dilation, self.groups, self.padding_mode):
            return _GroupConvFn.apply(x, w, self.bias, self.stride[0], self.padding[0], self.dilation[0], self.groups)
        _warn_aten_fallback('Conv2d', x, f'weight {tuple(w.shape)}, stride {self.stride}, groups {self.groups}, '
                                           f'padding_mode {self.padding_mode}, input {tuple(x.shape)} {x.dtype}')
# ... 2 lines not shown
```

### lsnet_amd/ops/dcn.py

```python
import math

import torch
import torch.nn as nn
import torch.nn.functional as F
from torch.autograd import Function
from torch.autograd.function import once_differentiable
from torch.nn.modules.utils import _pair, _single

from ..cnn.registry import CONV_LAYERS
from . import grad_sink
from .backend import get_backend
from . import conv as _conv
from .conv import Conv2d


def _conv_out(size, k, stride, pad, dil):
    return (size + 2 * pad - (dil * (k - 1) + 1)) // stride + 1


def _same_int(v, what):
    v = _pair(v)
    if v[0] != v[1]:
        raise NotImplementedError(f'{what} must be the same for height and width, got {v}')
    return int(v[0])


def _backend_backward(ctx, inputs, offsets, masks, weight, gos, need):
    sinks_ok = getattr(ctx.backend, 'dcn_sinks_ok', None)
    c = grad_sink.claim([(weight, need['weight']), (ctx.bias_ref, need['bias'])], optional=(1,),
                        allowed=sinks_ok is not None and sinks_ok(inputs, weight))
    kw = dict(sinks=c.sinks) if c.accumulate else {}
    gxs, goffs, gmsks, gw, gb = ctx.backend.dcn_backward(inputs, offsets, masks, weight, gos, ctx.cfg, need, **kw)
    return (gxs, goffs, gmsks, *c.results((gw, gb)))


class _DCNFunction(Function):

    @staticmethod
    def forward(ctx, weight, bias, cfg, n, *tensors):
        inputs, offsets, masks = tensors[:n], tensors[n:2 * n], tensors[2 * n:3 * n]
        backend = get_backend(inputs[0])
        out_hw = []
        for x, off in zip(inputs, offsets):
            if cfg['pyramid']:
                hw = (_conv_out(off.shape[2], weight.shape[2], cfg['stride'], cfg['pad'], cfg['dil']),
                      _conv_out(off.shape[3], weight.shape[3], cfg['stride'], cfg['pad'], cfg['dil']))
            else:
                hw = (_conv_out(x.shape[2], weight.shape[2], cfg['stride'], cfg['pad'], cfg['dil']),
                      _conv_out(x.shape[3], weight.shape[3], cfg['stride'], cfg['pad'], cfg['dil']))
            if not all(s > 0 for s in hw):
                raise ValueError('convolution input is too small (output would be '
                                 f'{x.shape[0]}x{weight.shape[0]}x{hw[0]}x{hw[1]})')
            if tuple(off.shape[2:]) != hw:
                raise RuntimeError(f'invalid spatial size of offset, expected height: {hw[0]} width: {hw[1]}, '
                                   f'but got height: {off.shape[2]} width: {off.shape[3]}')
            if off.shape[1] != cfg['dg'] * (3 if cfg.get('fused_om') else 2) * weight.shape[2] * weight.shape[3]:
                raise RuntimeError('invalid number of channels of offset')
            out_hw.append(hw)
        ctx.cfg, ctx.n, ctx.backend = cfg, n, backend
        ctx.has_bias = bias is not None
        ctx.bias_ref = bias
        ctx.mask_none = [m is None for m in masks]
        ctx.save_for_backward(weight, *inputs, *offsets, *[m for m in masks if m is not None])
        outs = backend.dcn_forward(list(inputs), list(offsets), list(masks), weight, bias, cfg, out_hw)
        cat = int(cfg.get('concat') or 0)
        if cat > 1 and len(outs) == n:
            outs = [torch.cat(outs[j:j + cat], dim=1) for j in range(0, n, cat)]
        return tuple(outs)

    @staticmethod
    @once_differentiable
    def backward(ctx, *grad_outs):
        n, cfg = ctx.n, ctx.cfg
        saved = ctx.saved_tensors
        weight, inputs, offsets = saved[0], saved[1:1 + n], saved[1 + n:1 + 2 * n]
        rest = list(saved[1 + 2 * n:])
        masks = [None if none else rest.pop(0) for none in ctx.mask_none]
        nig = ctx.needs_input_grad
        need = dict(weight=nig[0], bias=ctx.has_bias and nig[1],
                    input=[nig[4 + i] for i in range(n)],
                    offset=[nig[4 + n + i] for i in range(n)],
                    mask=[nig[4 + 2 * n + i] for i in range(n)])
        gos = []
        cat = int(cfg.get('concat') or 0)
        if cat > 1:
            Co = weight.shape[0]
            for j, g in enumerate(grad_outs):
                x, off = inputs[j * cat], offsets[j * cat]
                if g is None:
                    g = x.new_zeros((x.shape[0], cat * Co, off.shape[2], off.shape[3]))
                if x.is_contiguous(memory_format=torch.channels_last):
                    g = g.contiguous(memory_format=torch.channels_last)
                gos += [g.narrow(1, q * Co, Co) for q in range(cat)]
        for i, g in enumerate(grad_outs if cat <= 1 else ()):
            if g is None:
                x, off = inputs[i], offsets[i]
                g = x.new_zeros((x.shape[0], weight.shape[0], off.shape[2], off.shape[3]))
            gos.append(g)
        gxs, goffs, gmsks, gw, gb = _backend_backward(ctx, list(inputs), list(offsets), masks, weight, gos, need)
        gxs = [g if need['input'][i] else None for i, g in enumerate(gxs)]
        goffs = [g if need['offset'][i] else None for i, g in enumerate(goffs)]
        gmsks = [g if (need['mask'][i] and not ctx.mask_none[i]) else None for i, g in enumerate(gmsks)]
        if gw is not None and gw.stride() != weight.stride():
            gw = gw.contiguous(memory_format=torch.channels_last if weight.is_contiguous(
                memory_format=torch.channels_last) and not weight.is_contiguous() else torch.contiguous_format)
        return (gw, gb, None, None, *gxs, *goffs, *gmsks)


class _DCNPackFn(Function):

    @staticmethod
    def forward(ctx, weight, bias, w_off, b_off, cfg, n, *xs):
        backend = get_backend(xs[0])
        pad, dil = cfg['pad'], cfg['dil']
        w_off = w_off.contiguous(memory_format=torch.channels_last)
        offs = _conv.conv_multi_fwd(xs, w_off, b_off, pad, dil, False)
        out_hw = [tuple(o.shape[2:]) for o in offs]
        outs = backend.dcn_forward(list(xs), offs, [None] * n, weight, bias, cfg, out_hw)
        ctx.cfg, ctx.n, ctx.backend = cfg, n, backend
        ctx.bias_ref, ctx.b_off_ref = bias, b_off
        ctx.save_for_backward(weight, w_off, *xs, *offs)
        return tuple(outs)

    @staticmethod
    @once_differentiable
    def backward(ctx, *grad_outs):
        n, cfg = ctx.n, ctx.cfg
        saved = ctx.saved_tensors
        weight, w_off, xs, offs = saved[0], saved[1], saved[2:2 + n], saved[2 + n:2 + 2 * n]
        nig = ctx.needs_input_grad
        need_x = [nig[6 + i] for i in range(n)]
        need_off = nig[2] or nig[3] or any(need_x)
        need = dict(weight=nig[0], bias=ctx.bias_ref is not None and nig[1], input=[True] * n if any(need_x) else [False] * n,
                    offset=[need_off] * n, mask=[False] * n)
        gos = [g if g is not None else x.new_zeros((x.shape[0], weight.shape[0], o.shape[2], o.shape[3]))
               for g, x, o in zip(grad_outs, xs, offs)]
        gxs, goffs, _, gw, gb = _backend_backward(ctx, list(xs), list(offs), [None] * n, weight, gos, need)
        pad, dil = cfg['pad'], cfg['dil']
        if any(need_x):
            gxs = _conv.conv_multi_dgrad(goffs, w_off, xs, pad, dil, accumulate_into=gxs)
        gwo = gbo = None
        if nig[2] or nig[3]:
            gwo, gbo = _conv.conv_multi_wgrad(xs, goffs, w_off, ctx.b_off_ref, pad, dil, nig[2], nig[3])
        return (gw, gb, gwo, gbo, None, None, *[g if nx else None for g, nx in zip(gxs, need_x)])


class _OffsetChainFn(Function):

    @staticmethod
    def forward(ctx, mults, copies, *offs):
        be = get_backend(offs[0])
        ctx.mults, ctx.be, ctx.device, ctx.copies = mults, be, offs[0].device, copies
        ctx.shapes = [tuple(o.shape) for o in offs]
        res = be.offset_chain(list(offs), mults)
        out = [t for trio in res for t in trio]
        if copies == 2:
            out += [t.view(t.shape) for t in out]
        return tuple(out)

    @staticmethod
    @once_differentiable
    def backward(ctx, *grads):
        n = len(ctx.shapes)
        gs = [list(grads[3 * l:3 * l + 3]) + (list(grads[3 * n + 3 * l:3 * n + 3 * l + 3]) if ctx.copies == 2 else [])
              for l in range(n)]
        return (None, None, *ctx.be.offset_chain_backward(ctx.shapes, ctx.device, ctx.mults, gs))


def offset_scale_chain(offs, mults, copies=1):
    offs = list(offs)
    if offs and all(o.is_cuda for o in offs) and len(offs) <= 8 and all(len(m) == 3 for m in mults) and copies in (1, 2):
        be = get_backend(offs[0])
        if all(be.offset_chain_ok(o) for o in offs):
            n = len(offs)
            flat = _OffsetChainFn.apply(tuple(tuple((float(a), float(b)) for a, b in m) for m in mults), copies, *offs)
            return [[list(flat[c * 3 * n + 3 * l:c * 3 * n + 3 * l + 3]) for l in range(n)] for c in range(copies)]
    res = []
    for off, m in zip(offs, mults):
        cur, trio = off, []
        for sh, sw in m:
            mult = _scale_const(float(sh), float(sw), off.shape[1], off.device, off.dtype)
            cur = cur * mult
            trio.append(cur)
        res.append(trio)
    return [res] * copies


_SCALE_CONSTS = {}


def _scale_const(sh, sw, channels, device, dtype):
    key = (sh, sw, channels, str(device), dtype)
    t = _SCALE_CONSTS.get(key)
    if t is None:
        t = torch.tensor([sh, sw], dtype=dtype).repeat(channels // 2).view(1, -1, 1, 1).to(device)
        _SCALE_CONSTS[key] = t
# ... 247 lines not shown
```

### lsnet_amd/ops/hip_backend.py

```python
import ctypes

import torch

from .. import _lib
from .._lib import ptr, stream
from .._lib import ptr as _ptr, stream as _stream
from .backend import register_backend

_CL = torch.channels_last
CACHE_DCN_IMAGES = __import__('os').environ.get('LSNET_CACHE_DCN_IMAGES', '1') != '0'


def _f32(t, what):
    if t.dtype != torch.float32:
        raise TypeError(f'{what} must be float32, got {t.dtype}')
    return t


def _is_nhwc(t):
    return t.dim() == 4 and t.is_contiguous(memory_format=_CL)


def _dense(t, nhwc):
    if t.is_contiguous() or t.is_contiguous(memory_format=_CL):
        return t
    return t.contiguous(memory_format=_CL) if nhwc else t.contiguous()


def _pixel_pitch(t):
    if t.dim() != 4 or t.stride(1) != 1:
        return None
    B, C, H, W = t.shape
    p = t.stride(3)
    if p < C or p % 4 or t.stride(2) != W * p or (B > 1 and t.stride(0) != H * W * p):
        return None
    return p


def pool_pitch(t):
    if t.dim() != 4 or (t.shape[1] > 1 and t.stride(1) != 1) or t.numel() == 0:
        return None
    B, C, H, W = t.shape
    p = t.stride(3) if W > 1 else t.stride(2) if H > 1 else t.stride(0) if B > 1 else C
    if p < C or (W > 1 and t.stride(3) != p) or (H > 1 and t.stride(2) != W * p) or (B > 1 and t.stride(0) != H * W * p):
        return None
    return p


def _writable(t):
    if t.dtype != torch.float32:
        return False
    expect = 1
    for st, n in sorted((st, n) for st, n in zip(t.stride(), t.shape) if n > 1):
        if st != expect:
            return False
        expect *= n
    return True


def _strides(t):
    s = t.stride()
    return _lib.Strides4(s[0], s[1], s[2], s[3])


class HipBackend:
    name = 'hip'

    @staticmethod
    def group_norm_supported(C, G):
        return C % 4 == 0 and C % G == 0 and ((C // G) % 4 == 0 or 4 % (C // G) == 0) and C // 4 <= 256 and 256 % (C // 4) == 0 and G <= 256

    @staticmethod
    def _gn_levels(xs, ys=None, dys=None, dxs=None):
        n = len(xs)
        levels = (_lib.GnLevel * n)()
        for i, x in enumerate(xs):
            B, C, H, W = x.shape
            L = levels[i]
            L.x = ptr(x)
            L.y = ptr(ys[i]) if ys is not None else None
            L.dy = ptr(dys[i]) if dys is not None else None
            L.dx = ptr(dxs[i]) if dxs is not None else None
            L.B, L.HW = B, H * W
        return levels

    def group_norm_forward(self, xs, gamma, beta, groups, eps, relu, cat_px=False):
        lib = _lib.load()
        n, C = len(xs), xs[0].shape[1]
        if cat_px:
            B = xs[0].shape[0]
            assert all(x.shape[0] == B for x in xs)
            hw = [x.shape[2] * x.shape[3] for x in xs]
            flat = torch.empty((B, sum(hw), C), device=xs[0].device, dtype=torch.float32)
            ys, o = [], 0
            for k in hw:
                ys.append(flat[:, o:o + k])
                o += k
            levels = self._gn_levels(xs, ys=ys)
            for L in levels:
                L.y_batch_stride = flat.stride(0)
        else:
            ys = [torch.empty_like(x, memory_format=_CL) for x in xs]
            levels = self._gn_levels(xs, ys=ys)
        images = sum(x.shape[0] for x in xs)
        mean_rstd = torch.empty(images, groups, 2, device=xs[0].device, dtype=torch.float32)
        ws = torch.empty(lib.lsn_group_norm_workspace_bytes(n, levels, C, groups), device=xs[0].device,
                         dtype=torch.uint8)
        _lib.check(lib.lsn_group_norm_forward(n, levels, C, groups, ptr(gamma), ptr(beta), eps, 1 if relu else 0,
                                              ptr(mean_rstd), ptr(ws), stream()))
        if cat_px:
            return flat.unsqueeze(2).permute(0, 3, 1, 2), mean_rstd
        return ys, mean_rstd

    supports_grad_sinks = True

    def group_norm_backward(self, xs, dys, gamma, beta, groups, relu, mean_rstd, need_params, sinks=None):
        lib = _lib.load()
        n, C = len(xs), xs[0].shape[1]
        dxs = [torch.empty_like(x, memory_format=_CL) for x in xs]
# ... 73 lines not shown
                    img = weight_image(w, 2 if backward else 0, 1, cfg['pad'], cfg['dil'])
                    shape.workspace = img.data_ptr()
                    return img
                except NotImplementedError:
                    pass
            shape.weights_prepared = 0
        ws = torch.empty(2 * w.numel(), device=w.device, dtype=torch.float32)
        shape.workspace = ws.data_ptr()
        return ws

    def dcn_forward(self, inputs, offsets, masks, weight, bias, cfg, out_hw):
        lib = _lib.load()
        nhwc, xs, offs, msks, w = self._prep(inputs, offsets, masks, weight)
        n = len(xs)
        shape = self._shape(w, cfg)
        levels = self._dcn_levels(xs, offs, msks, w, cfg, out_hw)
        outs = []
        g = int(cfg.get('concat') or 0)
        Co = w.shape[0]
        wide = None
        if g > 1:
            assert n % g == 0 and all(out_hw[i] == out_hw[i - i % g] and xs[i].shape[0] == xs[i - i % g].shape[0] for i in range(n))
            if nhwc and (g * Co) % 4 == 0:
                wide = [torch.empty((xs[j].shape[0], g * Co) + tuple(out_hw[j]), device=xs[j].device, dtype=torch.float32,
                                    memory_format=_CL) for j in range(0, n, g)]
        for i in range(n):
            if wide is not None:
                out = wide[i // g].narrow(1, (i % g) * Co, Co)
            else:
                out = torch.empty((xs[i].shape[0], Co) + tuple(out_hw[i]), device=xs[i].device, dtype=torch.float32,
                                  memory_format=_CL if nhwc else torch.contiguous_format)
            outs.append(out)
            levels[i].output = ptr(out)
        b = None if bias is None else _f32(bias.contiguous(), 'bias')
        if _lib.split_math():
            ws = self._weight_workspace(shape, levels, w, weight, cfg, nhwc, False)
        if wide is not None:
            shape.out_pitch = g * Co
            if not lib.lsn_dcn_pitched_ok(ctypes.byref(shape), n, levels, 0):
                shape.out_pitch = 0
                wide = None
                outs = [torch.empty(tuple(o.shape), device=o.device, dtype=torch.float32, memory_format=_CL) for o in outs]
                for i in range(n):
                    levels[i].output = ptr(outs[i])
        _lib.check(lib.lsn_dcn_forward(ctypes.byref(shape), n, levels, ptr(w), ptr(b), 1 if nhwc else 0, stream()))
        if g > 1:
            return wide if wide is not None else [torch.cat(outs[j:j + g], dim=1) for j in range(0, n, g)]
        return outs

    @staticmethod
    def dcn_sinks_ok(inputs, weight):
        return all(_is_nhwc(x) for x in inputs) and weight.is_contiguous(memory_format=_CL)

    def dcn_backward(self, inputs, offsets, masks, weight, grad_outs, cfg, need, sinks=None):
        nhwc, xs, offs, msks, w = self._prep(inputs, offsets, masks, weight)
        n = len(xs)
        pitches = {_pixel_pitch(g) for g in grad_outs} if nhwc else {None}
        if len(pitches) == 1 and None not in pitches and pitches != {w.shape[0]}:
            gos = list(grad_outs)
        else:
            gos = [(g.contiguous(memory_format=_CL) if nhwc else g.contiguous()) for g in grad_outs]
        gxs, goffs, gmsks = [], [], []
        shared = {}
        bufs = []
        for i in range(n):
            gx = gx_ret = None
            if need['input'][i]:
                key = (xs[i].data_ptr(), tuple(xs[i].shape)) if nhwc else i
                if key in shared:
                    gx = shared[key]
                else:
                    gx = gx_ret = shared[key] = torch.empty_like(xs[i])
            want_om = need['offset'][i] or (msks[i] is not None and need['mask'][i])
            goffs.append(torch.empty_like(offs[i]) if want_om else None)
            gmsks.append(torch.empty_like(msks[i]) if (want_om and msks[i] is not None) else None)
            gxs.append(gx_ret)
            bufs.append(gx)
        if sinks is not None:
            assert nhwc and w is weight, 'dcn_backward: sinks for a call that dcn_sinks_ok declines'
            gw, gb = sinks
            acc = 1
        else:
            gw = torch.empty_like(w) if (need['weight'] or need['bias']) else None
            gb = torch.empty(w.shape[0], device=w.device, dtype=torch.float32) if need['bias'] else None
            acc = 0
        self._dcn_backward_call(xs, offs, msks, w, gos, bufs, goffs, gmsks, gw, gb, acc, cfg, nhwc, weight)
        return gxs, goffs, gmsks, gw, gb

    def _dcn_backward_call(self, xs, offs, msks, w, gos, gx_bufs, goffs, gmsks, gw, gb, accumulate, cfg, nhwc, weight=None):
        lib = _lib.load()
        n = len(xs)
        shape = self._shape(w, cfg)
        levels = self._dcn_levels(xs, offs, msks, w, cfg, [g.shape[2:] for g in gos])
        for L, go, gx, goff, gmsk in zip(levels, gos, gx_bufs, goffs, gmsks):
            L.grad_output, L.grad_input, L.grad_offset, L.grad_mask = ptr(go), ptr(gx), ptr(goff), ptr(gmsk)
            if cfg.get('fused_om') and goff is not None:
                L.grad_mask = self._mask_view_ptr(goff, cfg, w.shape[2] * w.shape[3])
        nbytes = int(lib.lsn_dcn_backward_workspace_bytes(ctypes.byref(shape), n, levels))
        if nbytes > 0:
            gws = torch.empty(nbytes, device=w.device, dtype=torch.uint8)
            shape.gather_workspace, shape.gather_workspace_bytes = gws.data_ptr(), nbytes
        if cfg['groups'] == 1 and _lib.split_math():
            ws = self._weight_workspace(shape, levels, w, weight, cfg, nhwc, True)
        shape.accumulate_param_grads = 1 if accumulate else 0
        pitch = _pixel_pitch(gos[0]) if nhwc else None
        if pitch is not None and pitch != w.shape[0]:
            shape.out_pitch = pitch
            if not lib.lsn_dcn_pitched_ok(ctypes.byref(shape), n, levels, 1):
                shape.out_pitch = 0
                gos = [g.contiguous(memory_format=_CL) for g in gos]
                for i in range(n):
                    levels[i].grad_output = ptr(gos[i])
        _lib.check(lib.lsn_dcn_backward(ctypes.byref(shape), n, levels, ptr(w), ptr(gw), ptr(gb),
                                        1 if nhwc else 0, stream()))

    @staticmethod
    def _focal_rows(logits, targets, weight=None, d_losses=None):
        if logits.dim() != 2:
            raise ValueError(f'focal loss: logits must be (N, C), got {tuple(logits.shape)}')
        N, C = logits.shape
        if targets.dtype != torch.int64:
            raise TypeError('targets must be int64')
        if targets.numel() != N or targets.device != logits.device:
            raise ValueError(f'focal loss: {targets.numel()} targets on {targets.device} for {N} rows of logits on {logits.device}')
        if weight is not None and (weight.numel() != N or weight.device != logits.device):
            raise ValueError(f'focal loss: {weight.numel()} weights on {weight.device} for {N} rows of logits on {logits.device}')
        if d_losses is not None and (d_losses.shape != logits.shape or d_losses.device != logits.device):
            raise ValueError(f'focal loss: upstream gradient {tuple(d_losses.shape)} for logits {tuple(logits.shape)}')
        return N, C

    def focal_forward(self, logits, targets, gamma, alpha):
        lib = _lib.load()
        logits = _f32(logits, 'logits').contiguous()
        targets = targets.contiguous()
        if targets.dtype != torch.int64:
            raise TypeError('targets must be int64')
        out = torch.empty_like(logits)
        N, C = self._focal_rows(logits, targets)
        _lib.check(lib.lsn_sigmoid_focal_loss_forward(ptr(logits), ptr(targets), ptr(out), N, C, gamma, alpha,
                                                      stream()))
        return out

    def focal_backward(self, logits, targets, d_losses, gamma, alpha):
        lib = _lib.load()
        logits = logits.contiguous()
        d_losses = d_losses.contiguous()
        out = torch.empty_like(logits)
        N, C = self._focal_rows(logits, targets, d_losses=d_losses)
        _lib.check(lib.lsn_sigmoid_focal_loss_backward(ptr(logits), ptr(targets.contiguous()), ptr(d_losses),
                                                       ptr(out), N, C, gamma, alpha, stream()))
        return out

    def focal_sum(self, logits, targets, weight, gamma, alpha):
        lib = _lib.load()
        logits = _f32(logits, 'logits').contiguous()
        out = torch.empty((), device=logits.device, dtype=torch.float32)
        N, C = self._focal_rows(logits, targets, weight)
        w = None if weight is None else _f32(weight, 'weight').contiguous()
        _lib.check(lib.lsn_sigmoid_focal_loss_sum(ptr(logits), ptr(targets.contiguous()), ptr(w), ptr(out), N,
                                                  C, gamma, alpha, stream()))
        return out

    def focal_backward_weighted(self, logits, targets, weight, scale, gamma, alpha):
        lib = _lib.load()
        logits = logits.contiguous()
        out = torch.empty_like(logits)
        N, C = self._focal_rows(logits, targets, weight)
# ... 649 lines not shown
```

### lsnet_amd/ops/pool.py

```python
import os

import torch
import torch.nn.functional as F

from .backend import get_backend

_CL = torch.channels_last
NATIVE_POOL = os.environ.get('LSNET_NATIVE_POOL', '1') != '0'


def _pair(v):
    return list(v) if isinstance(v, (tuple, list)) else [v, v]


def _square(v):
    a, b = _pair(v)
    return int(a) if a == b and isinstance(a, int) else None


def _pitched(t):
    from .hip_backend import pool_pitch
    p = pool_pitch(t)
    return p is not None and p % 4 == 0 and t.data_ptr() % 16 == 0


def native_ok(*tensors):
    if not NATIVE_POOL:
        return False
    for t in tensors:
        if not (torch.is_tensor(t) and t.is_cuda and t.dtype == torch.float32 and t.dim() == 4 and t.numel() > 0
                and t.shape[1] % 4 == 0 and t.numel() < (1 << 33) and _pitched(t)):
            return False
    return True


def _grad_arg(g):
    return g if (g.dtype == torch.float32 and _pitched(g)) else g.float().clone(memory_format=_CL)


def _fallback(what, x, detail):
    if NATIVE_POOL:
        from .conv import _warn_aten_fallback
        _warn_aten_fallback(what, x, detail)


def _describe(*ts):
    return ', '.join(f'{tuple(t.shape)} {t.dtype} strides {t.stride()}' for t in ts)


class _MaxPoolFn(torch.autograd.Function):

    @staticmethod
    def forward(ctx, x, kernel, stride, pad):
        be = get_backend(x)
        need = ctx.needs_input_grad[0] and kernel != (1, 1)
        y, slot = be.max_pool2d_forward(x, kernel, stride, pad, want_slot=need)
        ctx.cfg = (tuple(x.shape), kernel, stride, pad)
# ... 36 lines not shown

    @staticmethod
    def backward(ctx, go):
        (xc,) = ctx.saved_tensors
        k, s, p, ceil_mode, count_include_pad = ctx.cfg
        gx = torch.ops.aten.avg_pool2d_backward(go.contiguous(), xc, _pair(k), _pair(s), _pair(p), ceil_mode,
                                                count_include_pad, None)
        return gx, None, None, None, None, None


def avg_pool_nchw(x, pool):
    s = pool.stride if pool.stride is not None else pool.kernel_size
    return _AvgPoolNCHW.apply(x, pool.kernel_size, s, pool.padding, bool(pool.ceil_mode), bool(pool.count_include_pad))


class _AvgPoolFn(torch.autograd.Function):

    @staticmethod
    def forward(ctx, x, kernel, stride, pad, ceil_mode, count_include_pad):
        ctx.cfg = (tuple(x.shape), kernel, stride, pad, ceil_mode, count_include_pad)
        return get_backend(x).avg_pool2d_forward(x, kernel, stride, pad, ceil_mode, count_include_pad)

    @staticmethod
    @torch.autograd.function.once_differentiable
    def backward(ctx, go):
        shape, kernel, stride, pad, ceil_mode, count_include_pad = ctx.cfg
        go = _grad_arg(go)
        gx = get_backend(go).avg_pool2d_backward(go, shape, kernel, stride, pad, ceil_mode, count_include_pad)
        return gx, None, None, None, None, None


def avg_pool2d(x, kernel_size, stride=None, padding=0, ceil_mode=False, count_include_pad=True):
    kernel = tuple(_pair(kernel_size))
    s, p = _square(kernel_size if stride is None else stride), _square(padding)
    if native_ok(x) and s is not None and p is not None and s > 0 and all(isinstance(k, int) and 2 * p <= k for k in kernel) \
            and kernel[0] * kernel[1] <= 255 and x.shape[2] + 2 * p >= kernel[0] and x.shape[3] + 2 * p >= kernel[1]:
        return _AvgPoolFn.apply(x, kernel, s, p, bool(ceil_mode), bool(count_include_pad))
    _fallback('avg_pool2d', x, f'window {kernel}, stride {stride}, padding {padding}, input {_describe(x)}')
    st = kernel_size if stride is None else stride
    return _AvgPoolNCHW.apply(x, kernel_size, st, padding, bool(ceil_mode), bool(count_include_pad))


def avg_pool(x, pool):
    if pool.divisor_override is not None:
        return avg_pool_nchw(x, pool)
    return avg_pool2d(x, pool.kernel_size, pool.stride, pool.padding, pool.ceil_mode, pool.count_include_pad)


class _UpsampleAddFn(torch.autograd.Function):

    @staticmethod
    def forward(ctx, top, lat):
        ctx.top_shape = tuple(top.shape)
        return get_backend(lat).upsample_add_forward(top, lat)

    @staticmethod
    @torch.autograd.function.once_differentiable
    def backward(ctx, go):
        g = _grad_arg(go)
        gt = get_backend(g).upsample_add_backward(g, ctx.top_shape) if ctx.needs_input_grad[0] else None
        return gt, (go if ctx.needs_input_grad[1] else None)


def upsample_add(top, lat, upsample_cfg=None):
    cfg = dict(mode='nearest') if upsample_cfg is None else dict(upsample_cfg)
    if set(cfg) == {'mode'} and cfg['mode'] == 'nearest' and native_ok(top, lat) and top.shape[:2] == lat.shape[:2] \
            and all(big in (2 * small, 2 * small - 1) for small, big in zip(top.shape[2:], lat.shape[2:])):
        return _UpsampleAddFn.apply(top, lat)
    if 'scale_factor' in cfg:
        return lat + F.interpolate(top, **cfg)
    _fallback('upsample_add', lat, f'{cfg}, top {_describe(top)}, lateral {_describe(lat)}')
    return lat + F.interpolate(top, size=lat.shape[2:], **cfg)
```

### lsnet_amd/ops/resblock.py

```python
import weakref

import torch

from . import conv as K

_live_queues = weakref.WeakSet()
_callback_armed = [False]


class WgQueue(dict):
    __slots__ = ('__weakref__',)
    __hash__ = object.__hash__

    def __eq__(self, other):
        return self is other


def pending_wgrad_jobs():
    return sum(len(v) for q in list(_live_queues) for v in q.values())


def reset_pending():
    _callback_armed[0] = False
    for q in list(_live_queues):
        q.clear()


def _flush_pending():
    _callback_armed[0] = False
    for q in list(_live_queues):
        if q:
            flush_wgrad_queue(q)


def _arm_flush_callback():
    if _callback_armed[0]:
        return
    try:
        torch.autograd.Variable._execution_engine.queue_callback(_flush_pending)
        _callback_armed[0] = True
    except RuntimeError:
        pass


def epilogue_ok(k, stride, pad, dil):
    for p in range(stride):
        if not any((p + pad - t * dil) % stride == 0 for t in range(k)):
            return False
    return True


def _cfg(conv):
    return conv.stride[0], conv.padding[0], conv.dilation[0]


class _BottleneckFn(torch.autograd.Function):

    @staticmethod
    def forward(ctx, x, blk, pregate_in, gy_pregated, wg_queue, wg_flush, *params):
        c1, c2, c3 = blk.conv1, blk.conv2, blk.conv3
        n1, n2, n3 = blk.norm1, blk.norm2, blk.norm3
        h1 = K.conv_fwd_bn(x, c1.weight, n1, *_cfg(c1), True)
        h2 = K.conv_fwd_bn(h1, c2.weight, n2, *_cfg(c2), True)
        if blk.downsample is not None:
            cd, nd = blk.downsample[-2], blk.downsample[-1]
            idt = K.conv_fwd_bn(x, cd.weight, nd, *_cfg(cd), False)
        else:
            idt = x
        y = K.conv_fwd_bn(h2, c3.weight, n3, *_cfg(c3), True, idt)
        ctx.save_for_backward(x, h1, h2, y)
        ctx.blk, ctx.flags = blk, (bool(pregate_in), bool(gy_pregated))
        ctx.wg = (wg_queue, bool(wg_flush))
        return y

    @staticmethod
    @torch.autograd.function.once_differentiable
    def backward(ctx, gy):
        x, h1, h2, y = ctx.saved_tensors
        blk = ctx.blk
        pregate_in, gy_pregated = ctx.flags
        c1, c2, c3 = blk.conv1, blk.conv2, blk.conv3
        n1, n2, n3 = blk.norm1, blk.norm2, blk.norm3
        need_x = ctx.needs_input_grad[0]
        gy = gy.contiguous(memory_format=torch.channels_last)
        g3 = gy if gy_pregated else K.relu_gate(gy, y)
        grads = []

        def fused_dgrad(g, conv, bn, in_shape, gate, residual=None, out=None):
            k = conv.kernel_size[0]
            s, p, d = _cfg(conv)
            if epilogue_ok(k, s, p, d):
                return K.dgrad(g, conv.weight, in_shape, s, p, d, bn=bn, residual=residual, gate=gate, out=out)
            r = K.dgrad(g, conv.weight, in_shape, s, p, d, bn=bn)
            if residual is not None:
                r = r.add_(residual)
            return K.relu_gate(r, gate) if gate is not None else r

        queue, flush = ctx.wg

        def wgrad(xin, g, conv, bn, slot=None):
            if queue is not None and slot is not None and getattr(K, 'wgrad_bn_deferrable', None) \
                    and K.wgrad_bn_deferrable(conv.weight, bn):
                key = (tuple(xin.shape), tuple(conv.weight.shape), _cfg(conv))
                queue.setdefault(key, []).append((xin, g, conv.weight, bn))
                if isinstance(queue, WgQueue):
                    _live_queues.add(queue)
                    _arm_flush_callback()
                return None, None, None
            return K.wgrad_bn(xin, g, conv.weight, bn, *_cfg(conv))

        g2 = fused_dgrad(g3, c3, n3, h2.shape, h2)
        grads.append(wgrad(h2, g3, c3, n3, 'conv3'))
        g1 = fused_dgrad(g2, c2, n2, h1.shape, h1)
        grads.insert(0, wgrad(h1, g2, c2, n2, 'conv2'))
        gx = None
        gd = None
        if blk.downsample is not None:
            cd, nd = blk.downsample[-2], blk.downsample[-1]
            if need_x:
                gx = K.dgrad(g3, cd.weight, x.shape, *_cfg(cd), bn=nd)
            gd = wgrad(x, g3, cd, nd)
        if need_x:
            res = gx if gx is not None else g3
            gx = fused_dgrad(g1, c1, n1, x.shape, x if pregate_in else None, residual=res, out=gx)
        grads.insert(0, wgrad(x, g1, c1, n1, 'conv1'))
        flat = [t for trip in grads for t in trip]
        if gd is not None:
            flat += list(gd)
        if flush and queue:
            flush_wgrad_queue(queue)
        return (gx, None, None, None, None, None) + tuple(flat)


def flush_wgrad_queue(queue):
    for key in list(queue):
        jobs = queue.pop(key)
        cfg = key[2]
        if len(jobs) > 1:
            K.wgrad_bn_jobs(jobs, *cfg)
        else:
            K.wgrad_bn(*jobs[0], *cfg)


def bottleneck_ok(blk):
    from torch.nn.modules.batchnorm import _BatchNorm
    pairs = [(blk.conv1, blk.norm1), (blk.conv2, blk.norm2), (blk.conv3, blk.norm3)]
    if blk.downsample is not None:
        mods = list(blk.downsample)
        if len(mods) != 2:
            return False
        pairs.append((mods[0], mods[1]))
    if getattr(blk, 'with_cp', False) or getattr(blk, 'with_dcn', False):
        return False
    for conv, bn in pairs:
        if type(conv) is not K.Conv2d or conv.bias is not None or conv.groups != 1 or conv.padding_mode != 'zeros':
            return False
        if not isinstance(bn, _BatchNorm) or bn.training or not bn.affine or not bn.track_running_stats:
            return False
        if not (conv.weight.requires_grad and bn.weight.requires_grad and bn.bias.requires_grad):
            return False
        Co, C, kh, kw = conv.weight.shape
        if C % 4 or Co % 4 or kh != kw or conv.stride[0] != conv.stride[1] or conv.padding[0] != conv.padding[1] \
                or conv.dilation[0] != conv.dilation[1] or not conv.weight.is_contiguous(memory_format=torch.channels_last):
            return False
    return True


def bottleneck(blk, x, pregate_in=False, gy_pregated=False, wg_queue=None, wg_flush=False):
    params = []
    pairs = [(blk.conv1, blk.norm1), (blk.conv2, blk.norm2), (blk.conv3, blk.norm3)]
    if blk.downsample is not None:
        pairs.append((blk.downsample[-2], blk.downsample[-1]))
    for conv, bn in pairs:
        params += [conv.weight, bn.weight, bn.bias]
    return _BottleneckFn.apply(x, blk, pregate_in, gy_pregated, wg_queue, wg_flush, *params)
```

Measured before the change: 70.15 img/s.

## Accumulate fan-out gradients in place across DCN, conv dgrad and upsample backward

Adds a grad_meet fan_out mechanism so a tensor consumed by several ops (backbone outputs, FPN laterals, head tower features) collects its input gradients in one channels_last buffer instead of autograd summing separate tensors. DCN gather backward kernels gain a grad_input_accumulate flag that read-modify-writes into the existing buffer. Conv dgrad and upsample_add backward write into the shared buffer through a residual/accumulate epilogue, and some dgrads are deferred until the meet point. The aim is to cut the extra gradient buffers and elementwise add kernels, in exchange for more Python bookkeeping per tensor and ordering-dependent state in autograd callbacks.

```diff
diff --git a/include/lsnet_hip.h b/include/lsnet_hip.h
--- a/include/lsnet_hip.h
+++ b/include/lsnet_hip.h
@@ -47,6 +47,7 @@
     lsn_strides4 off_st, mask_st;
     int B, H, W, Ho, Wo;
     float scale_h, scale_w;
+    int grad_input_accumulate;
 } lsn_dcn_level;
 
 const char *lsn_last_error(void);
@@ -69,6 +70,7 @@
 int64_t lsn_dcn_backward_workspace_bytes(const lsn_dcn_shape *shape, int n_levels, const lsn_dcn_level *levels);
 int lsn_dcn_pitched_ok(const lsn_dcn_shape *shape, int n_levels, const lsn_dcn_level *levels, int backward);
 int lsn_dcn_prepared_ok(const lsn_dcn_shape *shape, int n_levels, const lsn_dcn_level *levels, int backward);
+int lsn_dcn_accumulate_ok(const lsn_dcn_shape *shape, int n_levels, const lsn_dcn_level *levels);
 int lsn_dcn_anchor_lists(const lsn_dcn_shape *shape, int n_levels, const lsn_dcn_level *levels, lsn_layout layout,
                          int *sample_anchor, int *list_start, int *list_sample, int64_t *counts, lsn_stream_t stream);
 
diff --git a/lsnet_amd/_lib.py b/lsnet_amd/_lib.py
--- a/lsnet_amd/_lib.py
+++ b/lsnet_amd/_lib.py
@@ -29,7 +29,8 @@
                 ('grad_offset', ctypes.c_void_p), ('grad_mask', ctypes.c_void_p),
                 ('off_st', Strides4), ('mask_st', Strides4),
                 ('B', ctypes.c_int), ('H', ctypes.c_int), ('W', ctypes.c_int), ('Ho', ctypes.c_int),
-                ('Wo', ctypes.c_int), ('scale_h', ctypes.c_float), ('scale_w', ctypes.c_float)]
+                ('Wo', ctypes.c_int), ('scale_h', ctypes.c_float), ('scale_w', ctypes.c_float),
+                ('grad_input_accumulate', ctypes.c_int)]
 
 
 class OffsetChainLevel(ctypes.Structure):
@@ -144,6 +145,7 @@
         'lsn_dcn_backward_workspace_bytes': (q, [P(DcnShape), i, P(DcnLevel)]),
         'lsn_dcn_pitched_ok': (i, [P(DcnShape), i, P(DcnLevel), i]),
         'lsn_dcn_prepared_ok': (i, [P(DcnShape), i, P(DcnLevel), i]),
+        'lsn_dcn_accumulate_ok': (i, [P(DcnShape), i, P(DcnLevel)]),
         'lsn_dcn_anchor_lists': (i, [P(DcnShape), i, P(DcnLevel), i, p, p, p, p, p]),
         'lsn_deform_conv_forward': (i, [p] * 4 + [i] * 16 + [p]),
         'lsn_deform_conv_backward_input': (i, [p] * 6 + [i] * 16 + [p]),
diff --git a/lsnet_amd/csrc/dcn.hip b/lsnet_amd/csrc/dcn.hip
--- a/lsnet_amd/csrc/dcn.hip
+++ b/lsnet_amd/csrc/dcn.hip
@@ -312,7 +312,8 @@
 static size_t gather_ws_bytes(const lsn_dcn_shape &s) { return (size_t)(s.gather_workspace_bytes > 0 ? s.gather_workspace_bytes : 0); }
 static bool aligned16(const void *p) { return (reinterpret_cast<uintptr_t>(p) & 15) == 0; }
 
-static DcnRouteShape route_shape(const DcnArgs &a, const lsn_dcn_shape &s, lsn_layout layout, bool want_wgrad)
+static DcnRouteShape route_shape(const DcnArgs &a, const lsn_dcn_shape &s, lsn_layout layout, bool want_wgrad,
+                                 const lsn_dcn_level *lv = nullptr)
 {
     DcnRouteShape r = {};
     r.n = a.nlv;
@@ -324,6 +325,7 @@
         R.x_aligned16 = aligned16(L.x), R.gout_aligned16 = aligned16(L.gout);
         R.gx_id = 0;
         while (a.lv[R.gx_id].gx != L.gx) ++R.gx_id;
+        R.gx_acc = R.gx && lv != nullptr && lv[i].grad_input_accumulate != 0;
     }
     const int K = a.kh * a.kw, KD = K * a.dg;
     r.C = a.C, r.Co = a.Co, r.kh = a.kh, r.kw = a.kw, r.groups = a.groups, r.dg = a.dg, r.SL = a.SL, r.opitch = a.opitch;
@@ -349,11 +351,11 @@
     aa.ncb = pl.ncb, aa.hb_slot = pl.hb_slot;
     for (int j = 0; j < pl.nblk; ++j) {
         const GatherPlanGroup &G = pl.blk[j];
-        ga.g[j] = GatherGrp{a.lv[G.level].gx, a.lv[G.level].x, G.B, G.H, G.W, G.abase, G.first};
+        ga.g[j] = GatherGrp{a.lv[G.level].gx, a.lv[G.level].x, G.B, G.H, G.W, G.abase, G.first, G.acc ? 1 : 0};
     }
     for (int j = 0; j < pl.nanc; ++j) {
         const GatherPlanGroup &G = pl.anc[j];
-        aa.g[j] = AnchorGrp{a.lv[G.level].gx, a.lv[G.level].x, G.B, G.H, G.W, G.abase, G.first};
+        aa.g[j] = AnchorGrp{a.lv[G.level].gx, a.lv[G.level].x, G.B, G.H, G.W, G.abase, G.first, G.acc ? 1 : 0};
     }
 }
 
@@ -823,7 +825,12 @@
     a.gb = grad_bias;
 
     void *gws = s.gather_workspace;
-    const DcnRoute r = route_backward(route_shape(a, s, layout, a.gw != nullptr));
+    const DcnRoute r = route_backward(route_shape(a, s, layout, a.gw != nullptr, lv));
+    if (r.acc_disagree)
+        return fail(LSN_ERR_INVALID, "deformable backward: levels that share a grad_input buffer disagree on grad_input_accumulate");
+    if (r.acc_asked && !r.accumulate_ok)
+        return fail(LSN_ERR_UNSUPPORTED, "deformable backward: grad_input_accumulate outside the atomic-free gather routes "
+                    "(lsn_dcn_accumulate_ok)");
     if (r.lds_over)
         return fail(LSN_ERR_UNSUPPORTED, "deformable backward: kh*kw*deformable_groups = %d needs %zu B of LDS (> 160 KiB) in the "
                     "fp32 scatter kernel, the only one left for this call; every call with at most %d is served",
@@ -1016,6 +1023,13 @@
     DcnRouteShape rs;
     if (!query_shape(rs, shape, n_levels, levels, backward, false)) return 0;
     return (backward ? route_backward(rs) : route_forward(rs)).prepared ? 1 : 0;
+}
+
+int lsn_dcn_accumulate_ok(const lsn_dcn_shape *shape, int n_levels, const lsn_dcn_level *levels)
+{
+    DcnRouteShape rs;
+    if (!query_shape(rs, shape, n_levels, levels, 1, false)) return 0;
+    return route_backward(rs).accumulate_ok ? 1 : 0;
 }
 
 int lsn_dcn_pitched_ok(const lsn_dcn_shape *shape, int n_levels, const lsn_dcn_level *levels, int backward)
diff --git a/lsnet_amd/csrc/dcn_gather_kernels.h b/lsnet_amd/csrc/dcn_gather_kernels.h
--- a/lsnet_amd/csrc/dcn_gather_kernels.h
+++ b/lsnet_amd/csrc/dcn_gather_kernels.h
@@ -15,6 +15,7 @@
     int B, H, W;
     int abase;
     int blk0;
+    int acc;
 };
 struct GatherArgs {
     GatherGrp g[MAXLV];
@@ -33,6 +34,7 @@
     int B, H, W;
     int abase;
     int a0;
+    int acc;
 };
 struct AnchorArgs {
     AnchorGrp g[MAXLV];
@@ -460,7 +462,12 @@
                             r.x = (r.x + r2.x) + (r1.x + r3.x), r.y = (r.y + r2.y) + (r1.y + r3.y);
                             r.z = (r.z + r2.z) + (r1.z + r3.z), r.w = (r.w + r2.w) + (r1.w + r3.w);
                         }
-                        *reinterpret_cast<float4 *>(G.gx + ((size_t)(b * G.H + y0 + i) * G.W + x0 + j) * C + c) = r;
+                        float4 *gp = reinterpret_cast<float4 *>(G.gx + ((size_t)(b * G.H + y0 + i) * G.W + x0 + j) * C + c);
+                        if (G.acc) {
+                            const float4 o = *gp;
+                            r.x = o.x + r.x, r.y = o.y + r.y, r.z = o.z + r.z, r.w = o.w + r.w;
+                        }
+                        *gp = r;
                     }
         }
         if constexpr (NW == 4) __syncthreads();
@@ -613,7 +620,12 @@
         float4 r;
         r.x = ((s11.x + s10.x) + s01.x) + s00.x, r.y = ((s11.y + s10.y) + s01.y) + s00.y;
         r.z = ((s11.z + s10.z) + s01.z) + s00.z, r.w = ((s11.w + s10.w) + s01.w) + s00.w;
-        *reinterpret_cast<float4 *>(G.gx + ((size_t)(b * G.H + y) * G.W + x) * ga.C + c) = r;
+        float4 *gp = reinterpret_cast<float4 *>(G.gx + ((size_t)(b * G.H + y) * G.W + x) * ga.C + c);
+        if (G.acc) {
+            const float4 o = *gp;
+            r.x = o.x + r.x, r.y = o.y + r.y, r.z = o.z + r.z, r.w = o.w + r.w;
+        }
+        *gp = r;
     }
 }
 
diff --git a/lsnet_amd/csrc/dcn_route.h b/lsnet_amd/csrc/dcn_route.h
--- a/lsnet_amd/csrc/dcn_route.h
+++ b/lsnet_amd/csrc/dcn_route.h
@@ -18,6 +18,7 @@
     bool gx, goff, gmsk;
     bool x_aligned16, gout_aligned16;
     int gx_id;
+    bool gx_acc = false;
 };
 
 struct DcnRouteShape {
@@ -140,6 +141,7 @@
     int B, H, W;
     int abase;
     int first;
+    bool acc = false;
 };
 
 struct GatherPlan {
@@ -179,7 +181,7 @@
             if (grp[j].level == L.gx_id) gi = j;
         if (gi < 0) {
             gi = ng++;
-            grp[gi] = GatherPlanGroup{i, L.B, L.H, L.W, (int)anchors, (int)Q};
+            grp[gi] = GatherPlanGroup{i, L.B, L.H, L.W, (int)anchors, (int)Q, L.gx_acc};
             anchors += (int64_t)L.B * (L.H + 1) * (L.W + 1);
             Q += (int64_t)L.B * dr_cdiv(L.H, DR_GT) * dr_cdiv(L.W, DR_GT);
         } else if (grp[gi].B != L.B || grp[gi].H != L.H || grp[gi].W != L.W) {
@@ -284,6 +286,9 @@
     int fp32_bn = 0;
     int fp32_red = 0;
     size_t lds_over = 0;
+    bool accumulate_ok = false;
+    bool acc_asked = false;
+    bool acc_disagree = false;
     GatherPlan plan;
     bool gather() const { return data == GATHER_GROUPED || data == GATHER_MM || data == GATHER_XN; }
 };
@@ -359,6 +364,12 @@
         }
         r.image = r.data == GATHER_MM ? IMG_FRAGMENT : can_split ? IMG_PLANES_T : IMG_NONE;
         r.prepared = !s.nchw && r.data == GATHER_MM;
+        r.accumulate_ok = !s.nchw && r.gather();
+        for (int i = 0; i < s.n; ++i) {
+            if (!s.lv[i].gx) continue;
+            r.acc_asked = r.acc_asked || s.lv[i].gx_acc;
+            r.acc_disagree = r.acc_disagree || s.lv[i].gx_acc != s.lv[s.lv[i].gx_id].gx_acc;
+        }
     }
     if (s.want_wgrad) {
         int64_t rows = 0, steps = 0;
diff --git a/lsnet_amd/models/backbones/resnet.py b/lsnet_amd/models/backbones/resnet.py
--- a/lsnet_amd/models/backbones/resnet.py
+++ b/lsnet_amd/models/backbones/resnet.py
@@ -9,6 +9,7 @@
 from ...ops.batch_norm import bn_act
 from ...ops import resblock
 from ...ops.conv import conv_bn_act, conv_bn_act_frozen
+from ...ops.grad_meet import fan_out
 from ...ops.pool import avg_pool, max_pool
 from ..builder import BACKBONES
 
@@ -284,7 +285,11 @@
         for i, name in enumerate(self.res_layers):
             x = getattr(self, name)(x)
             if i in self.out_indices:
-                outs.append(x)
+                if i + 1 < len(self.res_layers):
+                    x, out = fan_out(x, 2, defer_dgrad=(1,))
+                    outs.append(out)
+                else:
+                    outs.append(x)
         return tuple(outs)
 
     def train(self, mode=True):
diff --git a/lsnet_amd/models/dense_heads/ls_head.py b/lsnet_amd/models/dense_heads/ls_head.py
--- a/lsnet_amd/models/dense_heads/ls_head.py
+++ b/lsnet_amd/models/dense_heads/ls_head.py
@@ -12,6 +12,7 @@
 from ...ops.backend import get_backend
 from ...ops import ModulatedDeformConvPack, PyramidDeformConv
 from ...ops.dcn import offset_scale_chain
+from ...ops.grad_meet import fan_out
 from ...ops import cross_iou as fused_ciou
 from ...ops import point_decode as point_ops
 from ...ops.focal import level_rows_ok, level_sums
@@ -300,10 +301,12 @@
         nl = len(feats)
         shapes = [tuple(f.shape[2:]) for f in feats]
         base_offset = self._base_offset(feats[0])
-        cls_feats = self._run_tower(self.cls_convs, feats)
+        feats_for = list(zip(*[fan_out(f, 1 + len(self.branches)) for f in feats]))
+        cls_feats = self._run_tower(self.cls_convs, feats_for[0])
+        cls_feats, cls_feats_conv = zip(*[fan_out(f, 2) for f in cls_feats])
         st = {}
-        for b in self.branches:
-            tower = self._run_tower(getattr(self, f'{b}_convs'), feats)
+        for bi, b in enumerate(self.branches):
+            tower, tower_gather, tower_conv = zip(*[fan_out(f, 3) for f in self._run_tower(getattr(self, f'{b}_convs'), feats_for[1 + bi])])
             init_conv, init_out = getattr(self, f'pts_{b}_init_conv'), getattr(self, f'pts_{b}_init_out')
             n_sp = self._out_dims(b)[1]
             raw = init_out(self._cat_px(init_conv.forward_multi(tower, relu=True)))
@@ -314,7 +317,8 @@
                 reg = self.get_pred_reg(sp, raw[:, n_sp:] if raw.shape[1] > n_sp else None)
                 reg = (1 - self.gradient_mul) * reg.detach() + self.gradient_mul * reg
                 off = reg - base_offset
-            st[b] = dict(feat=tower, sp_all=sp, sp=self._split_px(sp, shapes), off=self._split_px(off, shapes))
+            st[b] = dict(feat=tower_gather, feat_conv=tower_conv, sp_all=sp, sp=self._split_px(sp, shapes),
+                         off=self._split_px(off, shapes))
 
         if after_init is not None:
             after_init({b: st[b]['sp'] for b in self.branches})
@@ -350,13 +354,13 @@
             f = fc.forward_multi(feat)
             return [x + y for x, y in zip(a, f)]
 
-        fused = fuse(self.cls_af_dcn_conv, self.cls_feat_conv, cls_raw, cls_feats)
+        fused = fuse(self.cls_af_dcn_conv, self.cls_feat_conv, cls_raw, cls_feats_conv)
         outs['cls'] = self._split_px(self.pts_cls_out(self._gn_cat(self.cls_GN, fused)), shapes)
         for b in self.branches:
             raw = gather(getattr(self, f'pts_{b}_refine_conv'), st[b]['feat'], scaled[b])
             af, fc = getattr(self, f'{b}_af_dcn_conv'), getattr(self, f'{b}_feat_conv')
             gn, ro = getattr(self, f'{b}_GN'), getattr(self, f'pts_{b}_refine_out')
-            fused = fuse(af, fc, raw, st[b]['feat'])
+            fused = fuse(af, fc, raw, st[b]['feat_conv'])
             ref_raw, sp_init = ro(self._gn_cat(gn, fused)), st[b]['sp_all'].detach()
             if point_ops.native_ok(ref_raw, sp_init):
                 refine = point_ops.softplus_add(ref_raw, sp_init)
diff --git a/lsnet_amd/models/necks/fpn.py b/lsnet_amd/models/necks/fpn.py
--- a/lsnet_amd/models/necks/fpn.py
+++ b/lsnet_amd/models/necks/fpn.py
@@ -2,6 +2,7 @@
 import torch.nn.functional as F
 
 from ...cnn import ConvModule, xavier_init
+from ...ops.grad_meet import fan_out
 from ...ops.pool import max_pool2d, upsample_add
 from ..builder import NECKS
 
@@ -57,17 +58,22 @@
 
     def forward(self, inputs):
         assert len(inputs) == len(self.in_channels)
+        inputs, extra_src = list(inputs), None
+        if self.num_outs > len(self.lateral_convs) and self.add_extra_convs == 'on_input':
+            inputs[self.backbone_end_level - 1], extra_src = fan_out(inputs[self.backbone_end_level - 1], 2)
         lat = [conv(inputs[i + self.start_level]) for i, conv in enumerate(self.lateral_convs)]
         n = len(lat)
+        lat_out = list(lat)
         for i in range(n - 1, 0, -1):
-            lat[i - 1] = upsample_add(lat[i], lat[i - 1], self.upsample_cfg)
-        outs = [self.fpn_convs[i](lat[i]) for i in range(n)]
+            top, lat_out[i] = fan_out(lat[i], 2)
+            lat[i - 1] = lat_out[i - 1] = upsample_add(top, lat[i - 1], self.upsample_cfg)
+        outs = [self.fpn_convs[i](lat_out[i]) for i in range(n)]
         if self.num_outs > n:
             if not self.add_extra_convs:
                 for _ in range(self.num_outs - n):
                     outs.append(max_pool2d(outs[-1], 1, stride=2))
             else:
-                src = {'on_input': inputs[self.backbone_end_level - 1], 'on_lateral': lat[-1],
+                src = {'on_input': extra_src if extra_src is not None else inputs[self.backbone_end_level - 1], 'on_lateral': lat[-1],
                        'on_output': outs[-1]}[self.add_extra_convs]
                 outs.append(self.fpn_convs[n](src))
                 for i in range(n + 1, self.num_outs):
diff --git a/lsnet_amd/ops/conv.py b/lsnet_amd/ops/conv.py
--- a/lsnet_amd/ops/conv.py
+++ b/lsnet_amd/ops/conv.py
@@ -6,7 +6,7 @@
 
 from .. import _lib
 from .._lib import ptr, stream
-from . import grad_sink
+from . import grad_meet, grad_sink
 from .weight_images import SIDE_STREAM_IMAGES, _fold_bn, invalidate_weight_images, parameters_updated, weight_image
 
 _CL = torch.channels_last
@@ -161,6 +161,30 @@
     return _forward_prepared(x, img, shift, w.shape, stride, pad, dil, relu, residual)
 
 
+def _epilogue_ok(k, stride, pad, dil):
+    return all(any((p + pad - t * dil) % stride == 0 for t in range(k)) for p in range(stride))
+
+
+def _meet_dgrad(h, last, g, w, in_shape, stride, pad, dil, bn=None):
+    if h is None:
+        return dgrad(g, w, in_shape, stride, pad, dil, bn=bn)
+    can_add = in_shape[1] % 4 == 0 and w.shape[2] == w.shape[3] and _epilogue_ok(w.shape[2], stride, pad, dil)
+
+    def run():
+        buf = grad_meet.channels_last_buffer(h, in_shape) if can_add else None
+        if buf is not None:
+            dgrad(g, w, in_shape, stride, pad, dil, bn=bn, residual=buf, out=buf)
+            h.added()
+        else:
+            h.deliver(dgrad(g, w, in_shape, stride, pad, dil, bn=bn))
+
+    if last and can_add and h.partial() is None:
+        h.defer(run)
+    else:
+        run()
+    return None
+
+
 class _ConvFn(torch.autograd.Function):
 
     @staticmethod
@@ -170,6 +194,7 @@
         ctx.save_for_backward(x, w, out if relu else None)
         ctx.cfg = (stride, pad, dil, relu, bias is not None)
         ctx.bias_ref = bias
+        ctx.meet, ctx.meet_last = grad_meet.handle_of(x), grad_meet.wants_last(x)
         return out
 
     @staticmethod
@@ -186,7 +211,7 @@
         gx = gw = gb = None
         if ctx.needs_input_grad[0]:
             w8, (go8,), _ = _pad_narrow_co(w, [go])
-            gx = dgrad(go8, w8, x.shape, stride, pad, dil)
+            gx = _meet_dgrad(ctx.meet, ctx.meet_last, go8, w8, x.shape, stride, pad, dil)
         if ctx.needs_input_grad[1] or (has_bias and ctx.needs_input_grad[2]):
             want_b = has_bias and ctx.needs_input_grad[2]
             c, gw, gb = _param_grad_buffers(w, ctx.bias_ref, ctx.needs_input_grad[1], want_b)
@@ -274,11 +299,12 @@
     levels = (_lib.ConvLevel * n)()
     gxs = []
     for i, x in enumerate(xs):
-        gx = accumulate_into[i] if accumulate_into is not None else torch.empty_like(x, memory_format=_CL)
+        acc = accumulate_into[i] if accumulate_into is not None else None
+        gx = acc if acc is not None else torch.empty_like(x, memory_format=_CL)
         gxs.append(gx)
         L = levels[i]
         L.x, L.out, L.B, L.H, L.W = ptr(gos8[i]), ptr(gx), x.shape[0], x.shape[2], x.shape[3]
-        if accumulate_into is not None:
+        if acc is not None:
             L.residual = ptr(gx)
     _lib.check(_lib.load().lsn_conv2d_backward_data_prepared(n, levels, ptr(weight_image(w8, 1, 1, pad, dil)), C, Co8, kh, kw, 1,
                                                              pad, dil, stream()))
@@ -312,6 +338,7 @@
         ctx.save_for_backward(w, *xs, *(outs if relu else []))
         ctx.cfg, ctx.n, ctx.has_bias, ctx.nres = (pad, dil, relu), len(xs), bias is not None, nres
         ctx.bias_ref = bias
+        ctx.meet = [grad_meet.handle_of(x) for x in xs]
         return tuple(outs)
 
     @staticmethod
@@ -332,7 +359,13 @@
         need_x = [ctx.needs_input_grad[3 + i] for i in range(n)]
         gxs = [None] * n
         if any(need_x):
-            gxs = [g if need else None for g, need in zip(conv_multi_dgrad(gos, w, xs, pad, dil), need_x)]
+            meet = [h if need else None for h, need in zip(ctx.meet, need_x)]
+            into = [None if h is None else grad_meet.channels_last_buffer(h, x.shape) for h, x in zip(meet, xs)]
+            gxs = conv_multi_dgrad(gos, w, xs, pad, dil, into if any(t is not None for t in into) else None)
+            for i, h in enumerate(meet):
+                if h is not None:
+                    h.added() if into[i] is not None else h.deliver(gxs[i])
+            gxs = [g if need and h is None else None for g, need, h in zip(gxs, need_x, meet)]
         gw = gb = None
         if ctx.needs_input_grad[0] or (ctx.has_bias and ctx.needs_input_grad[1]):
             gw, gb = conv_multi_wgrad(xs, gos, w, ctx.bias_ref, pad, dil, ctx.needs_input_grad[0],
@@ -425,6 +458,7 @@
         ctx.save_for_backward(x, w, out if relu else None)
         ctx.cfg = (stride, pad, dil, relu, residual is not None)
         ctx.bn = bn
+        ctx.meet, ctx.meet_last = grad_meet.handle_of(x), grad_meet.wants_last(x)
         return out
 
     @staticmethod
@@ -439,7 +473,7 @@
         g = relu_gate(gy, y) if relu else gy
         gx = gw = dg = db = None
         if need_x:
-            gx = dgrad(g, w, x.shape, stride, pad, dil, bn=bn)
+            gx = _meet_dgrad(ctx.meet, ctx.meet_last, g, w, x.shape, stride, pad, dil, bn=bn)
         if need_w or need_g or need_b:
             gw, dg, db = wgrad_bn(x, g, w, bn, stride, pad, dil, (need_w, need_g, need_b))
         return gx, gw, dg, db, (g if need_res else None), None, None, None, None, None
diff --git a/lsnet_amd/ops/dcn.py b/lsnet_amd/ops/dcn.py
--- a/lsnet_amd/ops/dcn.py
+++ b/lsnet_amd/ops/dcn.py
@@ -8,7 +8,7 @@
 from torch.nn.modules.utils import _pair, _single
 
 from ..cnn.registry import CONV_LAYERS
-from . import grad_sink
+from . import grad_meet, grad_sink
 from .backend import get_backend
 from . import conv as _conv
 from .conv import Conv2d
@@ -25,11 +25,13 @@
     return int(v[0])
 
 
-def _backend_backward(ctx, inputs, offsets, masks, weight, gos, need):
+def _backend_backward(ctx, inputs, offsets, masks, weight, gos, need, accumulate_into=None):
     sinks_ok = getattr(ctx.backend, 'dcn_sinks_ok', None)
     c = grad_sink.claim([(weight, need['weight']), (ctx.bias_ref, need['bias'])], optional=(1,),
                         allowed=sinks_ok is not None and sinks_ok(inputs, weight))
     kw = dict(sinks=c.sinks) if c.accumulate else {}
+    if accumulate_into is not None and any(t is not None for t in accumulate_into):
+        kw['accumulate_into'] = accumulate_into
     gxs, goffs, gmsks, gw, gb = ctx.backend.dcn_backward(inputs, offsets, masks, weight, gos, ctx.cfg, need, **kw)
     return (gxs, goffs, gmsks, *c.results((gw, gb)))
 
@@ -62,6 +64,7 @@
         ctx.bias_ref = bias
         ctx.mask_none = [m is None for m in masks]
         ctx.save_for_backward(weight, *inputs, *offsets, *[m for m in masks if m is not None])
+        ctx.meet = [grad_meet.handle_of(x) for x in inputs]
         outs = backend.dcn_forward(list(inputs), list(offsets), list(masks), weight, bias, cfg, out_hw)
         cat = int(cfg.get('concat') or 0)
         if cat > 1 and len(outs) == n:
@@ -97,8 +100,14 @@
                 x, off = inputs[i], offsets[i]
                 g = x.new_zeros((x.shape[0], weight.shape[0], off.shape[2], off.shape[3]))
             gos.append(g)
-        gxs, goffs, gmsks, gw, gb = _backend_backward(ctx, list(inputs), list(offsets), masks, weight, gos, need)
-        gxs = [g if need['input'][i] else None for i, g in enumerate(gxs)]
+        meet = [h if need['input'][i] and getattr(ctx.backend, 'dcn_accumulate', False) else None for i, h in enumerate(ctx.meet)]
+        all_cl = all(x.is_contiguous(memory_format=torch.channels_last) for x in inputs)
+        into = [grad_meet.channels_last_buffer(h, x.shape) if h is not None and all_cl else None for h, x in zip(meet, inputs)]
+        gxs, goffs, gmsks, gw, gb = _backend_backward(ctx, list(inputs), list(offsets), masks, weight, gos, need, into)
+        for i, h in enumerate(meet):
+            if h is not None and gxs[i] is not None:
+                h.added() if into[i] is not None else h.deliver(gxs[i])
+        gxs = [g if need['input'][i] and meet[i] is None else None for i, g in enumerate(gxs)]
         goffs = [g if need['offset'][i] else None for i, g in enumerate(goffs)]
         gmsks = [g if (need['mask'][i] and not ctx.mask_none[i]) else None for i, g in enumerate(gmsks)]
         if gw is not None and gw.stride() != weight.stride():
@@ -120,6 +129,7 @@
         ctx.cfg, ctx.n, ctx.backend = cfg, n, backend
         ctx.bias_ref, ctx.b_off_ref = bias, b_off
         ctx.save_for_backward(weight, w_off, *xs, *offs)
+        ctx.meet = [grad_meet.handle_of(x) for x in xs]
         return tuple(outs)
 
     @staticmethod
@@ -142,6 +152,10 @@
         gwo = gbo = None
         if nig[2] or nig[3]:
             gwo, gbo = _conv.conv_multi_wgrad(xs, goffs, w_off, ctx.b_off_ref, pad, dil, nig[2], nig[3])
+        for i, h in enumerate(ctx.meet):
+            if h is not None and need_x[i] and gxs[i] is not None:
+                h.deliver(gxs[i])
+                need_x[i] = False
         return (gw, gb, gwo, gbo, None, None, *[g if nx else None for g, nx in zip(gxs, need_x)])
 
 
diff --git a/lsnet_amd/ops/grad_meet.py b/lsnet_amd/ops/grad_meet.py
--- /dev/null
+++ b/lsnet_amd/ops/grad_meet.py
@@ -0,0 +1,128 @@
+import os
+
+import torch
+
+ENABLED = os.environ.get('LSNET_GRAD_MEET', '1') != '0'
+
+stats = dict(buffers=0, accumulated=0, torch_adds=0)
+
+
+def reset_stats():
+    for k in stats:
+        stats[k] = 0
+
+
+class Handle:
+    __slots__ = ('shape', 'stride', 'dtype', 'device', '_buffer', '_deferred', '_armed', '__weakref__')
+
+    def __init__(self, x):
+        self.shape, self.stride, self.dtype, self.device = tuple(x.shape), tuple(x.stride()), x.dtype, x.device
+        self._buffer = None
+        self._deferred = []
+        self._armed = False
+
+    def partial(self):
+        return self._buffer
+
+    def deliver(self, g):
+        if g is None:
+            return
+        if self._buffer is None:
+            self._buffer = g
+            stats['buffers'] += 1
+            self._arm()
+        else:
+            self._buffer.add_(g)
+            stats['torch_adds'] += 1
+
+    def added(self):
+        stats['accumulated'] += 1
+
+    def claim(self):
+        if self._buffer is not None:
+            stats['accumulated'] += 1
+            return self._buffer, True
+        self._buffer = torch.empty_strided(self.shape, self.stride, dtype=self.dtype, device=self.device)
+        stats['buffers'] += 1
+        self._arm()
+        return self._buffer, False
+
+    def defer(self, job):
+        self._deferred.append(job)
+        self._arm()
+
+    def _arm(self):
+        if self._armed:
+            return
+        try:
+            torch.autograd.Variable._execution_engine.queue_callback(self._clear)
+            self._armed = True
+        except RuntimeError:
+            pass
+
+    def _clear(self):
+        self._buffer = None
+        self._deferred = []
+        self._armed = False
+
+    def _finish(self, grads):
+        for g in grads:
+            if g is None:
+                continue
+            if self._buffer is None:
+                self._buffer = g
+                grads = None
+            elif grads is None:
+                self._buffer = self._buffer + g
+                stats['torch_adds'] += 1
+            else:
+                self._buffer.add_(g)
+                stats['torch_adds'] += 1
+        jobs, self._deferred = self._deferred, []
+        if jobs and grads is None:
+            self._buffer = self._buffer.clone()
+        for job in jobs:
+            job()
+        out = self._buffer
+        self._buffer = None
+        return out
+
+
+class _FanOut(torch.autograd.Function):
+
+    @staticmethod
+    def forward(ctx, x, n, handle):
+        ctx.handle = handle
+        ctx.set_materialize_grads(False)
+        return tuple(x.view_as(x) for _ in range(n))
+
+    @staticmethod
+    def backward(ctx, *grads):
+        return ctx.handle._finish(grads), None, None
+
+
+def fan_out(x, n, defer_dgrad=()):
+    if not (ENABLED and torch.is_tensor(x) and torch.is_grad_enabled() and x.requires_grad) or n < 2:
+        return (x,) * n
+    handle = Handle(x)
+    outs = _FanOut.apply(x, n, handle)
+    for i, o in enumerate(outs):
+        o._grad_meet = handle
+        o._grad_meet_last = i in defer_dgrad
+    return outs
+
+
+def wants_last(x):
+    return bool(getattr(x, '_grad_meet_last', False))
+
+
+def handle_of(x):
+    return getattr(x, '_grad_meet', None) if torch.is_tensor(x) else None
+
+
+def channels_last_buffer(h, shape):
+    buf = h.partial()
+    if buf is None or tuple(buf.shape) != tuple(shape) or buf.dtype != torch.float32 \
+            or not buf.is_contiguous(memory_format=torch.channels_last):
+        return None
+    return buf
diff --git a/lsnet_amd/ops/hip_backend.py b/lsnet_amd/ops/hip_backend.py
--- a/lsnet_amd/ops/hip_backend.py
+++ b/lsnet_amd/ops/hip_backend.py
@@ -65,6 +65,7 @@
 
 class HipBackend:
     name = 'hip'
+    dcn_accumulate = True
 
     @staticmethod
     def group_norm_supported(C, G):
@@ -244,7 +245,7 @@
     def dcn_sinks_ok(inputs, weight):
         return all(_is_nhwc(x) for x in inputs) and weight.is_contiguous(memory_format=_CL)
 
-    def dcn_backward(self, inputs, offsets, masks, weight, grad_outs, cfg, need, sinks=None):
+    def dcn_backward(self, inputs, offsets, masks, weight, grad_outs, cfg, need, sinks=None, accumulate_into=None):
         nhwc, xs, offs, msks, w = self._prep(inputs, offsets, masks, weight)
         n = len(xs)
         pitches = {_pixel_pitch(g) for g in grad_outs} if nhwc else {None}
@@ -255,12 +256,19 @@
         gxs, goffs, gmsks = [], [], []
         shared = {}
         bufs = []
+        acc_bufs = {}
         for i in range(n):
             gx = gx_ret = None
             if need['input'][i]:
                 key = (xs[i].data_ptr(), tuple(xs[i].shape)) if nhwc else i
+                into = accumulate_into[i] if accumulate_into is not None else None
                 if key in shared:
                     gx = shared[key]
+                    assert into is None or into is gx, 'dcn_backward: levels of one source map with different accumulate_into'
+                elif into is not None:
+                    assert nhwc and into.shape == xs[i].shape and into.dtype == torch.float32 and into.is_contiguous(memory_format=_CL)
+                    gx = gx_ret = shared[key] = into
+                    acc_bufs[id(into)] = into
                 else:
                     gx = gx_ret = shared[key] = torch.empty_like(xs[i])
             want_om = need['offset'][i] or (msks[i] is not None and need['mask'][i])
@@ -276,10 +284,11 @@
             gw = torch.empty_like(w) if (need['weight'] or need['bias']) else None
             gb = torch.empty(w.shape[0], device=w.device, dtype=torch.float32) if need['bias'] else None
             acc = 0
-        self._dcn_backward_call(xs, offs, msks, w, gos, bufs, goffs, gmsks, gw, gb, acc, cfg, nhwc, weight)
+        self._dcn_backward_call(xs, offs, msks, w, gos, bufs, goffs, gmsks, gw, gb, acc, cfg, nhwc, weight, acc_bufs)
         return gxs, goffs, gmsks, gw, gb
 
-    def _dcn_backward_call(self, xs, offs, msks, w, gos, gx_bufs, goffs, gmsks, gw, gb, accumulate, cfg, nhwc, weight=None):
+    def _dcn_backward_call(self, xs, offs, msks, w, gos, gx_bufs, goffs, gmsks, gw, gb, accumulate, cfg, nhwc, weight=None,
+                           acc_bufs=None):
         lib = _lib.load()
         n = len(xs)
         shape = self._shape(w, cfg)
@@ -303,8 +312,20 @@
                 gos = [g.contiguous(memory_format=_CL) for g in gos]
                 for i in range(n):
                     levels[i].grad_output = ptr(gos[i])
+        fresh = {}
+        if acc_bufs:
+            if nhwc and lib.lsn_dcn_accumulate_ok(ctypes.byref(shape), n, levels):
+                for L, gx in zip(levels, gx_bufs):
+                    L.grad_input_accumulate = 1 if (gx is not None and id(gx) in acc_bufs) else 0
+            else:
+                fresh = {k: torch.empty_like(t) for k, t in acc_bufs.items()}
+                for L, gx in zip(levels, gx_bufs):
+                    if gx is not None and id(gx) in fresh:
+                        L.grad_input = ptr(fresh[id(gx)])
         _lib.check(lib.lsn_dcn_backward(ctypes.byref(shape), n, levels, ptr(w), ptr(gw), ptr(gb),
                                         1 if nhwc else 0, stream()))
+        for k, t in fresh.items():
+            acc_bufs[k].add_(t)
 
     @staticmethod
     def _focal_rows(logits, targets, weight=None, d_losses=None):
diff --git a/lsnet_amd/ops/pool.py b/lsnet_amd/ops/pool.py
--- a/lsnet_amd/ops/pool.py
+++ b/lsnet_amd/ops/pool.py
@@ -3,6 +3,7 @@
 import torch
 import torch.nn.functional as F
 
+from . import grad_meet
 from .backend import get_backend
 
 _CL = torch.channels_last
@@ -145,13 +146,23 @@
     @staticmethod
     def forward(ctx, top, lat):
         ctx.top_shape = tuple(top.shape)
+        ctx.meet = grad_meet.handle_of(top)
         return get_backend(lat).upsample_add_forward(top, lat)
 
     @staticmethod
     @torch.autograd.function.once_differentiable
     def backward(ctx, go):
         g = _grad_arg(go)
-        gt = get_backend(g).upsample_add_backward(g, ctx.top_shape) if ctx.needs_input_grad[0] else None
+        gt = None
+        if ctx.needs_input_grad[0] and ctx.meet is not None:
+            buf = grad_meet.channels_last_buffer(ctx.meet, ctx.top_shape)
+            if buf is not None:
+                get_backend(g).upsample_add_backward(g, ctx.top_shape, out=buf, accumulate=True)
+                ctx.meet.added()
+            else:
+                ctx.meet.deliver(get_backend(g).upsample_add_backward(g, ctx.top_shape))
+        elif ctx.needs_input_grad[0]:
+            gt = get_backend(g).upsample_add_backward(g, ctx.top_shape)
         return gt, (go if ctx.needs_input_grad[1] else None)
 
 
diff --git a/lsnet_amd/ops/resblock.py b/lsnet_amd/ops/resblock.py
--- a/lsnet_amd/ops/resblock.py
+++ b/lsnet_amd/ops/resblock.py
@@ -3,6 +3,7 @@
 import torch
 
 from . import conv as K
+from . import grad_meet
 
 _live_queues = weakref.WeakSet()
 _callback_armed = [False]
@@ -71,6 +72,7 @@
         ctx.save_for_backward(x, h1, h2, y)
         ctx.blk, ctx.flags = blk, (bool(pregate_in), bool(gy_pregated))
         ctx.wg = (wg_queue, bool(wg_flush))
+        ctx.meet = grad_meet.handle_of(x)
         return y
 
     @staticmethod
@@ -129,6 +131,9 @@
             flat += list(gd)
         if flush and queue:
             flush_wgrad_queue(queue)
+        if ctx.meet is not None and gx is not None:
+            ctx.meet.deliver(gx)
+            gx = None
         return (gx, None, None, None, None, None) + tuple(flat)
 
 
```

New measurement: 70.32 img/s (median of 6 runs). No clear change (+0.2%).
